# Enigmatisms/NeRF

Hardware: AMD Instinct MI355X
Metric: rays/s (64+128 samples), 800x800 (higher is better)
Workload: dtype bf16

## Files before the change

include/nerf_amd.h:

```cpp
#ifndef NERF_AMD_H
#define NERF_AMD_H

#include <stddef.h>
#include <stdint.h>

#ifdef __cplusplus
extern "C" {
#endif

#define NERF_AMD_OK            0
#define NERF_AMD_EINVAL       -1
#define NERF_AMD_EUNSUPPORTED -2
#define NERF_AMD_EHIP         -3

#define NERF_AMD_F32   0
#define NERF_AMD_BF16  1
#define NERF_AMD_BF16_F8 2

#define NERF_AMD_NET_PROPOSAL 0
#define NERF_AMD_NET_MIP      1
#define NERF_AMD_NET_REF      2
#define NERF_AMD_NET_PROPOSAL_128 3
#define NERF_AMD_PROP_W128 0x100
#define NERF_AMD_NET_MIP_128 4
#define NERF_AMD_FINE_W128 0x200

#define NERF_AMD_ACT_RELU     0
#define NERF_AMD_ACT_IDENTITY 1
#define NERF_AMD_ACT_SOFTPLUS 2

const char* nerf_amd_last_error(void);
int         nerf_amd_version(void);
int         nerf_amd_device_info(int* n_cu, int* arch_is_gfx950);

typedef struct nerf_amd_samples {
    int32_t      mode;
    int32_t      S;
    int64_t      M;
    const float* pts;
    int32_t      pts_stride;
    int32_t      z_stride;
    const float* rays;
    const float* z;
    const float* z_base;
    const float* u;
    float        z_jitter;
    int32_t      H, W;
    float        fx, fy;
    float        pose[12];
    int32_t      contract;
    int32_t      ipe;
    float        ipe_radius;
    const float* ipe_dir_norm;
    uint64_t     rng_seed;
    int64_t      rng_ray_offset;
} nerf_amd_samples;

size_t nerf_amd_packed_bytes(int net, int precision);
int    nerf_amd_pack_weights(int net, int precision, const float* const* weights, const float* const* biases,
                             int n_tensors, void* packed, void* stream);

int nerf_amd_proposal_forward(const void* packed, int precision, const nerf_amd_samples* src,
                              float* density, void* stream);
int nerf_amd_mip_forward(const void* packed, int precision, const nerf_amd_samples* src,
                         float* rgbo, void* stream);

int nerf_amd_mip_forward_composite(const void* packed, int precision, const nerf_amd_samples* src, int white_bkg,
                                   float near, float far, float* rgb, float* depth, float* weights, void* stream);

#define NERF_AMD_REF_SRGB 1
int nerf_amd_ref_forward(const void* packed, int precision, const nerf_amd_samples* src, int ref_flags,
                         float* rgbo, float* normal, void* stream);
int nerf_amd_ref_forward_train(const void* packed, int precision, const nerf_amd_samples* src, int ref_flags, const float* bn_noise,
                               float* rgbo, float* normal, void* stream);


int nerf_amd_positional_encoding(const float* x, int64_t M, int L, float* out, void* stream);

int nerf_amd_ipe_feature(const float* z, const float* rays, int64_t N, int S, int L, float r, const float* dir_norm,
                         float* feat, float* mu, float* mu_t, void* stream);
int nerf_amd_ipe_feature_contracted(const float* z, const float* rays, int64_t N, int S, int L, float r, const float* dir_norm,
                                    float* feat, float* mu, float* mu_t, void* stream);
int nerf_amd_cone_parameters(const float* z, int64_t N, int S, float r, float* mu_t, float* var_t, float* var_r, void* stream);
int nerf_amd_dirs_norm(const float* rays, int64_t N, float* out, void* stream);

int nerf_amd_generate_rays(const float* pose_host, int H, int W, float fx, float fy, int64_t ray_offset, int64_t N,
                           float* rays, void* stream);

int nerf_amd_length2pts(const float* rays, const float* z, int64_t N, int S, float* out, void* stream);

int nerf_amd_sigma_to_weights(const float* sigma, const float* z, const float* dirs, int64_t N, int S, int act,
                              float* w, void* stream);

int nerf_amd_max_blur(const float* w, int64_t N, int S, float alpha, float* out, void* stream);

int nerf_amd_inverse_sample(const float* w, const float* z, const float* u, int64_t N, int C, int K, int sort,
                            float* z_out, int64_t* below, void* stream);

int nerf_amd_sample_pdf(const float* bins, const float* weights, const float* u, int64_t N, int B, int K, float* samples,
                        int64_t* below, int64_t* above, void* stream);

int nerf_amd_pixel_rays(const float* pose_host, float fx, float fy, const int64_t* coords, int64_t N, float* rays, void* stream);

int nerf_amd_sample_training_rays(const float* rgbs, const int64_t* coords, int64_t n_pixels, const float* pose_host, float fx, float fy,
                                  float near, float far, int64_t N, int C, uint64_t rng_seed, float* pts, float* lengths, float* rgb,
                                  float* rays, void* stream);
int nerf_amd_sample_training_rays_dev(const float* rgbs, const int64_t* coords, int64_t n_pixels, const float* pose_dev, float fx, float fy,
                                      float near, float far, int64_t N, int C, const uint64_t* seed_dev, float* pts, float* lengths,
                                      float* rgb, float* rays, void* stream);
int nerf_amd_philox_uniforms(float* out, int64_t N, int K, uint64_t rng_seed, const uint64_t* seed_dev, void* stream);
int nerf_amd_sample_scene_rays(const float* images, const float* poses, int64_t V, int H, int W, const int64_t* view_ids, int64_t K, int x0,
                               int x1, int y0, int y1, float fx, float fy, float near, float far, int64_t N, int C, uint64_t rng_seed,
                               const uint64_t* seed_dev, float* pts, float* lengths, float* rgb, float* rays, int64_t* index, void* stream);
#define NERF_AMD_PHILOX_INV 0
#define NERF_AMD_PHILOX_STRAT 1
int nerf_amd_philox_stream(float* out, int64_t N, int K, uint64_t rng_seed, const uint64_t* seed_dev, int64_t ray_offset, int stream_id,
// ... 151 lines not shown
```

nerf_amd/_lib.py:

```python
import ctypes as C
import os

import torch

_HERE = os.path.dirname(os.path.abspath(__file__))
LIB_PATH = os.environ.get("NERF_AMD_LIB") or os.path.join(_HERE, "libnerf_amd.so")

F32, BF16 = 0, 1
BF16_F8 = 2
EXPECTED_VERSION = 125
NET_PROPOSAL, NET_MIP, NET_REF, NET_PROPOSAL_128, NET_MIP_128 = 0, 1, 2, 3, 4
FINE_W128 = 0x200
PROP_W128 = 0x100
ACT_RELU, ACT_IDENTITY, ACT_SOFTPLUS = 0, 1, 2
SPACING_LINEAR, SPACING_DISPARITY = 0, 1
SPACINGS = {"linear": SPACING_LINEAR, "disparity": SPACING_DISPARITY}

c_float_p = C.POINTER(C.c_float)
c_void = C.c_void_p
i64 = C.c_int64


class Samples(C.Structure):
    _fields_ = [("mode", C.c_int32), ("S", C.c_int32), ("M", C.c_int64), ("pts", c_void), ("pts_stride", C.c_int32),
                ("z_stride", C.c_int32), ("rays", c_void), ("z", c_void), ("z_base", c_void), ("u", c_void),
                ("z_jitter", C.c_float), ("H", C.c_int32), ("W", C.c_int32), ("fx", C.c_float), ("fy", C.c_float),
                ("pose", C.c_float * 12), ("contract", C.c_int32), ("ipe", C.c_int32), ("ipe_radius", C.c_float),
                ("ipe_dir_norm", c_void), ("rng_seed", C.c_uint64), ("rng_ray_offset", C.c_int64)]


SIGNATURES = {
    "nerf_amd_last_error": (C.c_char_p, []),
    "nerf_amd_version": (C.c_int, []),
    "nerf_amd_device_info": (C.c_int, [C.POINTER(C.c_int), C.POINTER(C.c_int)]),
    "nerf_amd_packed_bytes": (C.c_size_t, [C.c_int, C.c_int]),
    "nerf_amd_pack_weights": (C.c_int, [C.c_int, C.c_int, C.POINTER(c_void), C.POINTER(c_void), C.c_int, c_void, c_void]),
    "nerf_amd_proposal_forward": (C.c_int, [c_void, C.c_int, C.POINTER(Samples), c_void, c_void]),
    "nerf_amd_mip_forward": (C.c_int, [c_void, C.c_int, C.POINTER(Samples), c_void, c_void]),
    "nerf_amd_mip_forward_composite": (C.c_int, [c_void, C.c_int, C.POINTER(Samples), C.c_int, C.c_float, C.c_float, c_void, c_void, c_void,
                                                 c_void]),
    "nerf_amd_ref_forward": (C.c_int, [c_void, C.c_int, C.POINTER(Samples), C.c_int, c_void, c_void, c_void]),
    "nerf_amd_ref_forward_train": (C.c_int, [c_void, C.c_int, C.POINTER(Samples), C.c_int, c_void, c_void, c_void, c_void]),
    "nerf_amd_positional_encoding": (C.c_int, [c_void, i64, C.c_int, c_void, c_void]),
    "nerf_amd_ipe_feature": (C.c_int, [c_void, c_void, i64, C.c_int, C.c_int, C.c_float, c_void, c_void, c_void, c_void, c_void]),
    "nerf_amd_ipe_feature_contracted": (C.c_int, [c_void, c_void, i64, C.c_int, C.c_int, C.c_float, c_void, c_void, c_void, c_void, c_void]),
    "nerf_amd_cone_parameters": (C.c_int, [c_void, i64, C.c_int, C.c_float, c_void, c_void, c_void, c_void]),
    "nerf_amd_dirs_norm": (C.c_int, [c_void, i64, c_void, c_void]),
    "nerf_amd_generate_rays": (C.c_int, [c_float_p, C.c_int, C.c_int, C.c_float, C.c_float, i64, i64, c_void, c_void]),
    "nerf_amd_length2pts": (C.c_int, [c_void, c_void, i64, C.c_int, c_void, c_void]),
    "nerf_amd_sigma_to_weights": (C.c_int, [c_void, c_void, c_void, i64, C.c_int, C.c_int, c_void, c_void]),
    "nerf_amd_max_blur": (C.c_int, [c_void, i64, C.c_int, C.c_float, c_void, c_void]),
    "nerf_amd_inverse_sample": (C.c_int, [c_void, c_void, c_void, i64, C.c_int, C.c_int, C.c_int, c_void, c_void, c_void]),
    "nerf_amd_sample_pdf": (C.c_int, [c_void, c_void, c_void, i64, C.c_int, C.c_int, c_void, c_void, c_void, c_void]),
    "nerf_amd_pixel_rays": (C.c_int, [c_float_p, C.c_float, C.c_float, c_void, i64, c_void, c_void]),
    "nerf_amd_sample_training_rays": (C.c_int, [c_void, c_void, i64, c_float_p, C.c_float, C.c_float, C.c_float, C.c_float, i64, C.c_int, C.c_uint64,
                                               c_void, c_void, c_void, c_void, c_void]),
    "nerf_amd_sample_training_rays_dev": (C.c_int, [c_void, c_void, i64, c_void, C.c_float, C.c_float, C.c_float, C.c_float, i64, C.c_int, c_void,
                                                   c_void, c_void, c_void, c_void, c_void]),
    "nerf_amd_sample_scene_rays": (C.c_int, [c_void, c_void, i64, C.c_int, C.c_int, c_void, i64, C.c_int, C.c_int, C.c_int, C.c_int, C.c_float, C.c_float,
                                            C.c_float, C.c_float, i64, C.c_int, C.c_uint64, c_void, c_void, c_void, c_void, c_void, c_void, c_void]),
    "nerf_amd_philox_uniforms": (C.c_int, [c_void, i64, C.c_int, C.c_uint64, c_void, c_void]),
    "nerf_amd_philox_stream": (C.c_int, [c_void, i64, C.c_int, C.c_uint64, c_void, i64, C.c_int, c_void]),
    "nerf_amd_advance_seed": (C.c_int, [c_void, c_void]),
    "nerf_amd_stratified_points": (C.c_int, [c_void, c_void, c_void, C.c_float, i64, C.c_int, c_void, c_void, c_void]),
    "nerf_amd_resample": (C.c_int, [c_void, c_void, c_void, c_void, C.c_float, c_void, C.c_int, c_void, i64, C.c_int,
                                    C.c_int, C.c_int, C.c_float, C.c_uint64, i64, c_void, c_void, c_void, c_void, c_void]),
    "nerf_amd_composite": (C.c_int, [c_void, c_void, C.c_int, c_void, C.c_int, i64, C.c_int, C.c_int, C.c_int, C.c_float, C.c_float,
                                     C.c_float, c_void, c_void, c_void, c_void, c_void, c_void, c_void]),
    "nerf_amd_train_dump_rows_mask_partials": (i64, []),
    "nerf_amd_train_dump_rows_mask": (C.c_int, [c_void, C.c_int, C.c_int, i64, C.c_int, C.c_int, c_void, c_void, c_void, c_void]),
    "nerf_amd_render_ref_workspace_bytes": (C.c_size_t, [i64, C.c_int]),
    "nerf_amd_render_rays_ref": (C.c_int, [c_void, c_void, C.c_int, C.c_int, c_void, C.POINTER(Samples), i64, c_void, c_void, c_void, i64, C.c_int,
                                          C.c_float, C.c_float, C.c_int, c_void, c_void, c_void, c_void, c_void, c_void]),
    "nerf_amd_encode_rows": (C.c_int, [c_void, C.c_int, i64, C.c_int, C.c_int, C.c_int, c_void, c_void]),
    "nerf_amd_merge_depths": (C.c_int, [c_void, c_void, i64, C.c_int, C.c_int, c_void, c_void]),
    "nerf_amd_merge_depths_order": (C.c_int, [c_void, c_void, c_void, i64, C.c_int, C.c_int, c_void, c_void, c_void, c_void]),
    "nerf_amd_coarse_grad_select": (C.c_int, [c_void, c_void, i64, C.c_int, C.c_int, C.c_int, c_void, c_void]),
    "nerf_amd_mfma_stream": (C.c_int, [C.c_int, C.c_int, C.c_int, c_void, c_void]),
    "nerf_amd_weighted_dot_loss": (C.c_int, [c_void, c_void, c_void, i64, C.c_int, C.c_float, c_void, c_void, c_void]),
    "nerf_amd_weighted_dot_loss_backward": (C.c_int, [c_void, c_void, c_void, c_void, i64, C.c_int, C.c_float, c_void, c_void, c_void, c_void]),
    "nerf_amd_distortion_loss": (C.c_int, [c_void, c_void, i64, C.c_int, C.c_int, C.c_float, c_void, c_void, c_void]),
    "nerf_amd_distortion_loss_backward": (C.c_int, [c_void, c_void, i64, C.c_int, C.c_int, C.c_float, c_void, c_void, c_void, c_void]),
    "nerf_amd_get_bounds": (C.c_int, [c_void, c_void, i64, C.c_int, C.c_int, c_void, c_void]),
    "nerf_amd_train_dump_bytes": (C.c_size_t, [C.c_int, C.c_int, i64]),
    "nerf_amd_proposal_forward_train": (C.c_int, [c_void, C.c_int, C.POINTER(Samples), c_void, c_void, c_void]),
    "nerf_amd_mip_forward_train": (C.c_int, [c_void, C.c_int, C.POINTER(Samples), c_void, c_void, c_void]),
    "nerf_amd_train_dump_to_rows": (C.c_int, [c_void, C.c_int, C.c_int, i64, C.c_int, C.c_int, c_void, c_void]),
    "nerf_amd_relu_mask": (C.c_int, [c_void, c_void, C.c_int, i64, c_void]),
    "nerf_amd_relu_mask_bias_partials": (i64, [C.c_int, i64, C.c_int]),
    "nerf_amd_relu_mask_bias": (C.c_int, [c_void, c_void, C.c_int, i64, C.c_int, c_void, c_void]),
    "nerf_amd_packed_backward_bytes": (C.c_size_t, [C.c_int, C.c_int]),
    "nerf_amd_pack_weights_backward": (C.c_int, [C.c_int, C.c_int, C.POINTER(c_void), C.c_int, c_void, c_void]),
    "nerf_amd_proposal_backward_chain": (C.c_int, [c_void, C.c_int, c_void, i64, c_void, c_void, c_void]),
    "nerf_amd_mip_backward_chain": (C.c_int, [c_void, C.c_int, c_void, c_void, i64, c_void, c_void, c_void]),
    "nerf_amd_weight_grads_workspace_bytes": (C.c_size_t, [C.c_int, C.c_int, i64]),
    "nerf_amd_proposal_weight_grads": (C.c_int, [C.c_int, i64, c_void, c_void, C.POINTER(c_void), C.POINTER(c_void), c_void, c_void]),
    "nerf_amd_mip_weight_grads": (C.c_int, [C.c_int, i64, c_void, c_void, C.POINTER(c_void), C.POINTER(c_void), C.POINTER(c_void),
                                           C.POINTER(c_void), c_void, c_void]),
    "nerf_amd_ref_forward_train_dump": (C.c_int, [c_void, C.c_int, C.POINTER(Samples), C.c_int, c_void, c_void, c_void, c_void, c_void, c_void]),
    "nerf_amd_ref_forward_train_dump_rng": (C.c_int, [c_void, C.c_int, C.POINTER(Samples), C.c_int, C.c_uint64, c_void, C.c_float, c_void, c_void, c_void,
                                                      c_void, c_void]),
    "nerf_amd_philox_normal": (C.c_int, [c_void, i64, C.c_uint64, c_void, C.c_float, i64, c_void]),
    "nerf_amd_density_grad_workspace_bytes": (C.c_size_t, [C.c_int, C.c_int, i64]),
    "nerf_amd_density_grad": (C.c_int, [C.c_int, c_void, C.c_int, i64, c_void, c_void, C.c_int, c_void, C.c_int, c_void, c_void, c_void]),
    "nerf_amd_ref_backward_workspace_bytes": (C.c_size_t, [C.c_int, i64]),
    "nerf_amd_ref_backward": (C.c_int, [c_void, C.c_int, C.c_int, i64, c_void, c_void, c_void, C.c_int, c_void, C.c_int, c_void, C.POINTER(c_void),
                                       C.POINTER(c_void), c_void, c_void]),
    "nerf_amd_adam_step": (C.c_int, [C.POINTER(c_void), C.POINTER(c_void), C.POINTER(c_void), C.POINTER(c_void), C.POINTER(i64), C.c_int, c_void,
                                    C.c_double, c_void, C.c_double, C.c_double, C.c_double, C.c_float, c_void]),
    "nerf_amd_sigma_to_weights_backward": (C.c_int, [c_void, c_void, c_void, i64, C.c_int, C.c_int, c_void, c_void, c_void]),
    "nerf_amd_composite_backward": (C.c_int, [c_void, c_void, C.c_int, c_void, C.c_int, i64, C.c_int, C.c_int, C.c_int, C.c_float, C.c_float,
                                              C.c_float, c_void, c_void, c_void, c_void, c_void]),
    "nerf_amd_max_blur_backward": (C.c_int, [c_void, c_void, i64, C.c_int, c_void, c_void]),
    "nerf_amd_get_bounds_backward": (C.c_int, [c_void, c_void, i64, C.c_int, C.c_int, c_void, c_void]),
    "nerf_amd_render_workspace_bytes": (C.c_size_t, [i64, C.c_int]),
    "nerf_amd_render_rays": (C.c_int, [c_void, c_void, C.c_int, c_void, C.POINTER(Samples), i64, c_void, c_void, c_void, i64,
                                       C.c_int, C.c_float, C.c_float, C.c_int, c_void, c_void, c_void, c_void, c_void]),
    "nerf_amd_warp_depths": (C.c_int, [c_void, c_void, i64, C.c_int, C.c_int, C.c_int, C.c_float, C.c_float, c_void, c_void, c_void]),
# ... 49 lines not shown
```

nerf_amd/_packed.py:

```python
from typing import List

import torch

from . import ops


class PackedWeightsMixin:

    _net_id: int = -1

    def _linear_layers(self) -> List[torch.nn.Linear]:
        raise NotImplementedError

    def _layers(self) -> List[torch.nn.Linear]:
        c = self.__dict__.get("_layers_cache")
        if c is None:
            c = self.__dict__["_layers_cache"] = list(self._linear_layers())
        return c

    def _layer_params(self):
        c = self.__dict__.get("_layer_params_cache")
        layers = self._layers()
        if c is None or c[0][0] is not layers[0].weight or c[1][-1] is not layers[-1].bias:
            c = self.__dict__["_layer_params_cache"] = ([l.weight for l in layers], [l.bias for l in layers])
        return c

    def _layers_changed(self) -> None:
        self.__dict__.pop("_layers_cache", None)
        self.__dict__.pop("_layer_params_cache", None)
        self.invalidate_packed()

    def _kernel_weight_shapes(self):
        return None

    def _column_segments(self):
        return None

    @staticmethod
    def encoding_segment(levels: int, cat_origin: bool, kernel_col: int = 0, module_col: int = 0):
        return (kernel_col, module_col, 3 + 6 * levels) if cat_origin else (kernel_col + 3, module_col, 6 * levels)

    def kernel_params(self, shapes=None):
        shapes = self._kernel_weight_shapes() if shapes is None else shapes
        ws, bs = self._layer_params()
        if shapes is None or all(tuple(w.shape) == tuple(s) for w, s in zip(ws, shapes)):
            return list(ws), list(bs)
        pw, pb = [], []
        segs = self._column_segments() or [None] * len(ws)
        with torch.no_grad():
            for w, b, s, seg in zip(ws, bs, shapes, segs):
                if tuple(w.shape) == tuple(s):
                    pw.append(w); pb.append(b)
                    continue
                W = torch.zeros(tuple(s), dtype=w.dtype, device=w.device)
                if seg is None:
                    W[: w.shape[0], : w.shape[1]] = w
                else:
                    for kc, mc, n in seg:
                        W[: w.shape[0], kc: kc + n] = w[:, mc: mc + n]
                B = torch.zeros((s[0],), dtype=b.dtype, device=b.device)
                B[: b.shape[0]] = b
                pw.append(W); pb.append(B)
        return pw, pb

    def unpad_grads(self, gW, gb):
        layers = self._layers()
        segs = self._column_segments() or [None] * len(layers)

        def cols(g, l, seg):
            if tuple(g.shape) == tuple(l.weight.shape):
                return g
            if seg is None:
                return g[: l.weight.shape[0], : l.weight.shape[1]]
            return torch.cat([g[: l.weight.shape[0], kc: kc + n] for kc, _, n in seg], dim=1)
        return ([cols(g, l, seg) for g, l, seg in zip(gW, layers, segs)],
                [g[: l.bias.shape[0]] if tuple(g.shape) != tuple(l.bias.shape) else g for g, l in zip(gb, layers)])

    def _generic(self) -> bool:
        return False

    def grad_sinks(self):
        owner = self.__dict__.get("_grad_owner")
        if owner is None or self._generic():
            return None
        layers = self._layers()
        shapes = self._kernel_weight_shapes()
        if shapes is not None and any(tuple(l.weight.shape) != tuple(sh) for l, sh in zip(layers, shapes)):
            return None
        return owner.sinks_for(self, layers)

    def _narrow_layout(self) -> bool:
        return False

    def _pack_now(self, precision: int, narrow: bool = False) -> torch.Tensor:
        ws, bs = self.kernel_params()
        return ops.pack_weights(self._net_id, precision, ws, bs)

    def packed_backward(self, precision: int) -> torch.Tensor:
        return ops.pack_weights_backward(self._net_id, precision, self.kernel_params()[0])

    def _packed_key(self):
        return (ops.PARAM_GENERATION[0],) + tuple((p.data_ptr(), p._version) for p in self.parameters())

    def invalidate_packed(self) -> None:
        self.__dict__.setdefault("_packed_cache", {}).clear()
        self.__dict__.setdefault("_rows_packed", {}).clear()

    def train(self, mode: bool = True):
        self.invalidate_packed()
        return super().train(mode)

    def packed(self, precision: int, wide: bool = False) -> torch.Tensor:
        narrow = (not wide) and self._narrow_layout()
        cache = self.__dict__.setdefault("_packed_cache", {})
        if self.training:
            cache.clear()
            return self._pack_now(precision, narrow)
        key = self._packed_key()
        hit = cache.get((precision, narrow))
        if hit is None or hit[0] != key:
            blob = self._pack_now(precision, narrow)
            cache[(precision, narrow)] = (key, blob)
            return blob
        return hit[1]


def require_no_grad(*tensors):
    if torch.is_grad_enabled() and any(t is not None and t.requires_grad for t in tensors):
        raise NotImplementedError(
            "nerf_amd: the HIP path is forward-only in this round (backward = SURVEY.md section 8f-1); "
            "wrap the call in torch.no_grad()")
```

nerf_amd/addtional.py:

```python
import torch
from torch import nn
from torch.nn import functional as F

from . import ops
from . import autograd_bridge as ab
from ._packed import PackedWeightsMixin, require_no_grad
from .nerf_helper import makeMLP


def getBounds(weights: torch.Tensor, inds: torch.Tensor):
    if ab.needs_grad(weights):
        return ab.HipOp.apply(lambda w, i: ops.get_bounds(w, i), lambda g, w, i: (ops.get_bounds_backward(i, g, w.shape[-1]), None), 1, weights, inds)
    return ops.get_bounds(weights, inds)


class ProposalLoss(nn.Module):
    def forward(self, prop_bounds: torch.Tensor, nerf_weights: torch.Tensor) -> torch.Tensor:
        return torch.sum(F.relu(nerf_weights - prop_bounds) ** 2 / (nerf_weights + 1e-8))


def _distortion(weights: torch.Tensor, t: torch.Tensor, mode: int, scale: float, expr) -> torch.Tensor:
    if not weights.is_cuda:
        return expr(weights, t) * scale
    if t.shape[-1] > ops.BWD_MAX_SAMPLES:
# ... 16 lines not shown
            dists = dists / dists.norm(dim=-1, keepdim=True)
            avg_weights = (weights[..., :-1] + weights[..., 1:]) / 2.
            delta = fine_ts[..., 1:] - fine_ts[..., :-1]
            return torch.mean(avg_weights[:, None, :] * avg_weights[..., None] * dists) + torch.mean(delta * (avg_weights ** 2)) / 3.
        return _distortion(weights, fine_ts, 0, 1.0, expr)


class DistortionLoss(nn.Module):

    def __init__(self, scale: float = 1.0) -> None:
        super().__init__()
        self.scale = float(scale)

    def forward(self, weights: torch.Tensor, edges: torch.Tensor) -> torch.Tensor:
        def expr(w, e):
            mid = (e[..., :-1] + e[..., 1:]) / 2.
            pair = (w[..., :, None] * w[..., None, :] * torch.abs(mid[..., :, None] - mid[..., None, :])).sum((-2, -1))
            return torch.mean(pair + (w * w * (e[..., 1:] - e[..., :-1])).sum(-1) / 3.)
        return _distortion(weights, edges, 1, self.scale, expr)


class SoftL1Loss(nn.Module):
    def __init__(self, epsilon=0.001) -> None:
        super().__init__()
        self.eps = epsilon

    def forward(self, pred: torch.Tensor, target: torch.Tensor):
        return torch.mean((pred - target) ** 2)


class LossPSNR(nn.Module):
    __LOG_10__ = 2.3025851249694824

    def forward(self, x):
        return -10. * torch.log(x) / LossPSNR.__LOG_10__


class ProposalNetwork(PackedWeightsMixin, nn.Module):
    _net_id = ops.NET_PROPOSAL
    _supports_grad_sinks = True

    @staticmethod
    def init_weight(m):
        if isinstance(m, nn.Linear):
            nn.init.trunc_normal_(m.weight, std=.02)
            if m.bias is not None:
                nn.init.constant_(m.bias, 0)

    def __init__(self, position_flevel, hidden_unit=128, cat_origin=True) -> None:
        super().__init__()
        self.position_dims = position_flevel * 6
        self.position_flevel = position_flevel
        self.cat_origin = cat_origin
        self.hidden_unit = hidden_unit
        in_dim = self.position_dims + (3 if cat_origin else 0)
        self.layers = nn.Sequential(*makeMLP(in_dim, hidden_unit), *makeMLP(hidden_unit, hidden_unit),
                                    *makeMLP(hidden_unit, hidden_unit), *makeMLP(hidden_unit, hidden_unit),
                                    *makeMLP(hidden_unit, 1, None))
        self.apply(self.init_weight)

    def _linear_layers(self):
        return [self.layers[0], self.layers[2], self.layers[4], self.layers[6], self.layers[8]]

    def _check_config(self):
        if not (self.position_flevel >= 1 and self.hidden_unit >= 1):
            raise NotImplementedError("nerf_amd: ProposalNetwork needs position_flevel >= 1 and hidden_unit >= 1")

    def _generic(self) -> bool:
        return self.hidden_unit > 256 or self.position_flevel > 10

    def _column_segments(self):
        if self.position_flevel == 10 and self.cat_origin:
            return None
        return [[self.encoding_segment(self.position_flevel, self.cat_origin)], None, None, None, None]

    def _kernel_weight_shapes(self):
        return [(256, 63), (256, 256), (256, 256), (256, 256), (1, 256)]

    _NARROW_SHAPES = [(128, 63), (128, 128), (128, 128), (128, 128), (1, 128)]

    def _narrow_layout(self) -> bool:
        return self.hidden_unit <= 128

    def _pack_now(self, precision: int, narrow: bool = False) -> torch.Tensor:
        if not narrow:
            return super()._pack_now(precision)
        ws, bs = self.kernel_params(self._NARROW_SHAPES)
        blob = ops.pack_weights(ops.NET_PROPOSAL_128, precision, ws, bs)
        blob._nerf_amd_layout = ops.PROP_W128
        return blob

    def loadFromFile(self, load_path: str, use_amp=False, other_stuff=None):
        save = torch.load(load_path, map_location="cpu")
        own = self.state_dict()
        own.update({k: save["model"][k] for k in own.keys()})
        self.load_state_dict(own)
        if use_amp:
            from apex import amp
            amp.load_state_dict(save["amp"])
        print("NeRF Model loaded from '%s'" % (load_path))
        if other_stuff is not None:
            return [save[k] for k in other_stuff]

    def forward(self, pts: torch.Tensor, encoded_pt: torch.Tensor = None, contract: bool = False) -> torch.Tensor:
        self._check_config()
        if self._generic():
            from . import generic_path
            return generic_path.proposal_forward(self, pts, contract=contract)
        prec = ops.current_precision()
        layers = self._layers()
        params = [l.weight for l in layers] + [l.bias for l in layers]
        if ab.needs_grad(pts, *params):
            if pts.numel() == 0:
                return ops.proposal_forward(self.packed(prec), prec, pts.detach(), contract=contract) + sum(q.sum() for q in params) * 0.0
            from . import mlp_backward
            held = {}
            tprec = prec if pts.requires_grad else ops.train_precision(prec)
            want_pos = bool(pts.requires_grad)

            def hip(p, *wb):
                out, held["dump"] = ops.proposal_forward_train(self.packed(prec, wide=True), tprec, p, contract=contract)
                return out

            def bwd(g, p, *wb):
                if "dump" not in held:
                    raise RuntimeError("nerf_amd: the activation dump of this forward was already consumed (backward twice over the same graph)")
                if "bwd_blob" not in held:
                    held["bwd_blob"] = self.packed_backward(prec)
                if ab._VJP.inputs_only:
                    gx = ops.density_grad(ops.NET_PROPOSAL, held["bwd_blob"], prec, held["dump"], p.reshape(-1, 3), scale=g.reshape(-1), contract=contract)
                    return (gx.view(p.shape), *[None] * len(wb))
                gx = None
                if ab.POSITION_GRADS and want_pos:
                    gx = ops.density_grad(ops.NET_PROPOSAL, held["bwd_blob"], prec, held["dump"], p.reshape(-1, 3), scale=g.reshape(-1), contract=contract).view(p.shape)
                sinks = self.grad_sinks()
                direct = sinks is not None and sinks[2]
                kw = wb[:5]
                gW, gb = mlp_backward.proposal_backward(g.reshape(-1), p.reshape(-1, 3), held.pop("dump"), tprec, kw, packed_bwd=held["bwd_blob"],
                                                        out=(sinks[0], sinks[1]) if direct else None)
                if sinks is not None:
                    if not direct:
                        torch._foreach_add_(list(sinks[0]) + list(sinks[1]), list(gW) + list(gb))
                    return (gx, *[None] * len(wb))
                gW, gb = self.unpad_grads(gW, gb)
                return (gx, *gW, *gb)
            return ab.HipOp.apply(hip, bwd, 1, pts, *params)
        return ops.proposal_forward(self.packed(prec), prec, pts, contract=contract)

    @staticmethod
    def get_weights(density: torch.Tensor, zvals: torch.Tensor, ray_dirs: torch.Tensor = None) -> torch.Tensor:
        if ab.needs_grad(density, zvals):
            if ray_dirs is not None:
                zvals = zvals * ray_dirs.norm(dim=-1, keepdim=True)
            if density.shape[-1] > ops.BWD_MAX_SAMPLES:
                ab.unsupported("a differentiable sigma -> weights row of %d samples (the backward kernel keeps a ray in registers: <= %d)" % (density.shape[-1], ops.BWD_MAX_SAMPLES))
            return ab.HipOp.apply(lambda s, z: ops.sigma_to_weights(s, z, None, ops.ACT_RELU),
                                  lambda g, s, z: (ops.sigma_to_weights_backward(s, z, None, ops.ACT_RELU, g), None), 1, density, zvals)
        return ops.sigma_to_weights(density, zvals, ray_dirs, ops.ACT_RELU)
```

nerf_amd/csrc/capi.hip:

```cpp
#include <hip/hip_runtime.h>
#include <stdio.h>
#include <string.h>

#include "../../include/nerf_amd.h"
#include "mlp_layout.h"

int mlp_launch_proposal(const void*, int, const nerf_amd_samples&, float*, hipStream_t);
int mlp_launch_proposal128(const void*, int, const nerf_amd_samples&, float*, hipStream_t);
int mlp_launch_mip(const void*, int, const nerf_amd_samples&, float*, hipStream_t);
int mlp_launch_mip128(const void*, int, const nerf_amd_samples&, float*, hipStream_t);
int mlp_launch_mip_composite(const void*, int, const nerf_amd_samples&, float*, float*, float*, int, float, float, hipStream_t);
int mlp_launch_ref(const void*, int, const nerf_amd_samples&, float*, float*, const float*, int, hipStream_t);
size_t mlp_train_layer_stride(int, int64_t);
size_t mlp_train_mask_stride(int, int64_t);
int mlp_launch_proposal_train(const void*, int, const nerf_amd_samples&, float*, void*, hipStream_t);
int mlp_launch_mip_train(const void*, int, const nerf_amd_samples&, float*, void*, hipStream_t);
int sk_frag_to_rows(const void*, int, int64_t, int, int64_t, void*, hipStream_t);
int sk_relu_mask(void*, const void*, int, int64_t, hipStream_t);
int sk_merge_sorted(const float*, const float*, int64_t, int, int, float*, hipStream_t);
int sk_merge_sorted_order(const float*, const float*, const int64_t*, int64_t, int, int, float*, int64_t*, int64_t*, hipStream_t);
int sk_coarse_grad_select(const float*, const int64_t*, int64_t, int, int, int, float*, hipStream_t);
int pack_mfma_stream(int, int, int, float*, hipStream_t);
int sk_weighted_dot_loss(const float*, const float*, const float*, int64_t, int, float, float*, float*, hipStream_t);
int sk_weighted_dot_loss_backward(const float*, const float*, const float*, const float*, int64_t, int, float, float*, float*, float*, hipStream_t);
int sk_distortion_loss(const float*, const float*, int64_t, int, int, float, float*, float*, hipStream_t);
int sk_distortion_loss_backward(const float*, const float*, int64_t, int, int, float, const float*, float*, float*, hipStream_t);
int sk_encode_rows(const float*, int, int64_t, int, int, int, void*, hipStream_t);
int sk_frag_rows_mask_blocks();
int sk_frag_rows_mask(const void*, int, int64_t, int, int64_t, void*, void*, float*, hipStream_t);
int sk_relu_mask_bias(void*, const void*, int, int64_t, int, float*, hipStream_t);
int pack_ref(int, const float* const*, const float* const*, void*, hipStream_t);
int pack_proposal_bwd(int, const float* const*, void*, hipStream_t);
int pack_mip_bwd(int, const float* const*, void*, hipStream_t);
int pack_ref_bwd(int, const float* const*, void*, hipStream_t);
int mlp_launch_ref_train(const void*, int, const nerf_amd_samples&, float*, float*, const float*, void*, float*, int, hipStream_t, unsigned long long, const unsigned long long*, float);
size_t bwd_density_grad_workspace_bytes(int, int64_t);
int bwd_density_grad(int, const void*, int, int64_t, const void*, const float*, int, const float*, int, float*, void*, hipStream_t, int);
size_t bwd_ref_workspace_bytes(int, int64_t);
int bwd_ref_backward(const void*, int, int64_t, const void*, const float*, const float*, int, const float*, int, const float*, float* const*,
                     float* const*, void*, int, hipStream_t);
int bwd_launch_prop_chain(const void*, int, const float*, int64_t, const void*, void*, hipStream_t);
int bwd_launch_mip_chain(const void*, int, const float*, const float*, int64_t, const void*, void*, hipStream_t);
size_t bwd_wgrad_workspace_bytes(int, int, int64_t);
int bwd_prop_weight_grads(int, int64_t, const void*, const void*, float* const*, float* const*, void*, hipStream_t);
int bwd_mip_weight_grads(int, int64_t, const void*, const void*, const float* const*, const float* const*, float* const*, float* const*, void*,
                         hipStream_t);
int bwd_launch_adam(float* const*, const float* const*, float* const*, float* const*, const long long*, int, float*, double, const double*, double,
                    double, double, float, hipStream_t);
int pack_proposal(int, const float* const*, const float* const*, void*, hipStream_t);
int pack_proposal128(int, const float* const*, const float* const*, void*, hipStream_t);
int pack_mip128(int, const float* const*, const float* const*, void*, hipStream_t);
int pack_mip(int, const float* const*, const float* const*, void*, hipStream_t);
int sk_positional_encoding(const float*, int64_t, int, float*, hipStream_t);
int sk_ipe_feature(const float*, const float*, int64_t, int, int, float, const float*, float*, float*, float*, int, hipStream_t);
int sk_dirs_norm(const float*, int64_t, float*, hipStream_t);
int sk_dirs_norm_scratch(const float*, int64_t, float*, void*, hipStream_t);
int sk_train_sampler(const float*, const int64_t*, int64_t, const float*, const float*, float, float, float, float, int64_t, int, uint64_t, const uint64_t*,
                     float*, float*, float*, float*, hipStream_t);
int sk_scene_sampler(const float*, const float*, int64_t, int, int, const int64_t*, int64_t, int, int, int, int, float, float, float, float, int64_t, int,
                     uint64_t, const uint64_t*, float*, float*, float*, float*, int64_t*, hipStream_t);
int sk_philox_uniforms(float*, int64_t, int, uint64_t, const uint64_t*, int64_t, int, hipStream_t);
int sk_philox_normal(float*, int64_t, uint64_t, const uint64_t*, float, int64_t, hipStream_t);
size_t gk_gemm_workspace_bytes(int64_t, int64_t, int64_t);
int gk_gemm(int, int64_t, int64_t, int64_t, const float*, int64_t, int64_t, const float*, int64_t, int64_t, float*, int64_t, const float*, int, const float*, int64_t,
            void*, hipStream_t);
int gk_sigmoid_backward(const float*, int64_t, const float*, int64_t, int64_t, int, float*, int64_t, hipStream_t);
int gr_dir_inputs(const float*, int64_t, const float*, int64_t, int64_t, int, const float*, float*, int64_t, float*, hipStream_t);
int gr_dir_inputs_backward(const float*, int64_t, const float*, int64_t, int64_t, int, const float*, const float*, int64_t, const float*, int64_t, float*, int64_t,
                           hipStream_t);
int gr_combine(const float*, int64_t, const float*, int64_t, int64_t, int, float*, hipStream_t);
int gr_combine_backward(const float*, int64_t, const float*, int64_t, const float*, int64_t, int64_t, int, float*, int64_t, float*, int64_t, hipStream_t);
int gr_pe_backward(const float*, int64_t, const float*, int64_t, int64_t, int, int, float*, hipStream_t);
int gr_add_rows(float*, int64_t, const float*, int64_t, int64_t, int, hipStream_t);
int gr_contract(const float*, int64_t, int64_t, const float*, int64_t, float*, hipStream_t);
int rg_rows_gemm(int64_t, int64_t, int64_t, const void*, int64_t, const void*, int64_t, int64_t, const float*, int, void*, int64_t, int, hipStream_t);
int rg_rows_to_bf16(const float*, int64_t, int64_t, int64_t, int, int, void*, int64_t, hipStream_t);
int sk_advance_seed(uint64_t*, hipStream_t);
int sk_cone_parameters(const float*, int64_t, int, float, float*, float*, float*, hipStream_t);
int sk_generate_rays(const float*, int, int, float, float, int64_t, int64_t, float*, hipStream_t);
int sk_length2pts(const float*, const float*, int64_t, int, float*, hipStream_t);
int sk_sigma_to_weights(const float*, const float*, const float*, int64_t, int, int, float*, hipStream_t);
int sk_max_blur(const float*, int64_t, int, float, float*, hipStream_t);
int sk_inverse_sample(const float*, const float*, const float*, int64_t, int, int, int, int, float*, int64_t*, int64_t*, hipStream_t);
int sk_pixel_rays(const float*, float, float, const int64_t*, int64_t, float*, hipStream_t);
int sk_stratified_points(const float*, const float*, const float*, float, int64_t, int, float*, float*, hipStream_t);
int sk_resample(const float*, const float*, const float*, const float*, float, const float*, int, const float*, int64_t, int,
                int, int, float, uint64_t, int64_t, float*, int64_t*, float*, float*, hipStream_t);
int sk_composite(const float*, const float*, int, const float*, int, int64_t, int, int, int, float, float, float, const float*,
                 const float*, float*, float*, float*, float*, hipStream_t);
int sk_get_bounds(const float*, const int64_t*, int64_t, int, int, float*, hipStream_t);
int sk_warp_depths(const float*, const float*, int64_t, int, int, float, float, float, float, float*, float*, hipStream_t);
int sk_warped_stratified(const float*, const float*, int64_t, int, uint64_t, int64_t, float, float, float, float, float*, float*, float*, hipStream_t);
size_t sk_warped_resample_lds_bytes(int, int);
int sk_warped_resample(const float*, const float*, const float*, int, const float*, int64_t, int, int, int, float, float, float, float, float, uint64_t,
                       int64_t, float*, float*, int64_t*, float*, hipStream_t);
int sk_weights_backward(const float*, int, int, const float*, int, const float*, int, int64_t, int, int, int, float, const float*, const float*,
                        const float*, const float*, int, float, float, float*, int, int, float*, hipStream_t);
int sk_max_blur_backward(const float*, const float*, int64_t, int, float*, hipStream_t);
int sk_get_bounds_backward(const int64_t*, const float*, int64_t, int, int, float*, hipStream_t);

namespace {
thread_local char g_err[512] = "";

int fail(int code, const char* fmt, const char* a = "") {
    snprintf(g_err, sizeof(g_err), fmt, a);
    return code;
}
int hip_status(int e, const char* where) {
    if (e == 0) return NERF_AMD_OK;
    snprintf(g_err, sizeof(g_err), "%s: HIP error %d (%s)", where, e, hipGetErrorString((hipError_t)e));
    return NERF_AMD_EHIP;
}
inline hipStream_t S(void* s) { return reinterpret_cast<hipStream_t>(s); }

int check_samples(const nerf_amd_samples* s, bool need_dir) {
    if (!s) return fail(NERF_AMD_EINVAL, "samples descriptor is NULL");
    if (s->M < 0) return fail(NERF_AMD_EINVAL, "negative sample count");
    if (s->mode == 0) {
        if (!s->pts && s->M) return fail(NERF_AMD_EINVAL, "mode 0 needs pts");
        if (s->pts_stride < (need_dir ? 6 : 3)) return fail(NERF_AMD_EINVAL, "pts_stride too small for this network");
    } else if (s->mode == 1 || s->mode == 2) {
        if (s->S <= 0) return fail(NERF_AMD_EINVAL, "S must be positive");
        if (s->mode == 1 && !s->rays && s->M) return fail(NERF_AMD_EINVAL, "mode 1 needs rays");
        if (s->mode == 2 && (s->H <= 0 || s->W <= 0)) return fail(NERF_AMD_EINVAL, "mode 2 needs H, W");
        if (!s->z && !s->z_base && s->M) return fail(NERF_AMD_EINVAL, "need z, or z_base (with u, or without: in-kernel uniforms from rng_seed)");
    } else {
        return fail(NERF_AMD_EINVAL, "unknown sample mode");
    }
    if (s->ipe) {
        if (!need_dir) return fail(NERF_AMD_EUNSUPPORTED, "integrated PE is wired for the MipNeRF kernel only");
        if (s->mode != 1 || !s->z || s->z_stride < s->S + 1) return fail(NERF_AMD_EINVAL, "integrated PE needs mode 1 with S+1 depths per ray (z, z_stride > S)");
        if (!s->ipe_dir_norm || !(s->ipe_radius > 0.0f)) return fail(NERF_AMD_EINVAL, "integrated PE needs ipe_dir_norm (device) and a positive ipe_radius");
    }
    return NERF_AMD_OK;
}
bool bad_prec(int p) { return p != NERF_AMD_F32 && p != NERF_AMD_BF16; }
int check_distortion(int64_t N, int Sn, int mode) {
    if (N < 0) return fail(NERF_AMD_EINVAL, "negative ray count");
    if (mode != 0 && mode != 1) return fail(NERF_AMD_EINVAL, "unknown mode (0: Regularizer, 1: Mip-NeRF 360 L_dist)");
    if (Sn < 2 || Sn > NERF_AMD_DISTORTION_MAX_S) return fail(NERF_AMD_EINVAL, "bad size (S must be 2..1024 depths per row: a ray's rows live in LDS)");
    return NERF_AMD_OK;
}
int check_spacing(int spacing, float near, float far, float* gn, float* gf) {
    if (spacing != NERF_AMD_SPACING_DISPARITY) return fail(NERF_AMD_EINVAL, "unknown spacing (the warped entry points take NERF_AMD_SPACING_DISPARITY only)");
    if (!(near > 0.0f)) return fail(NERF_AMD_EINVAL, "disparity spacing needs near > 0");
    if (!(far > near) || !(far <= 3.0e38f)) return fail(NERF_AMD_EINVAL, "disparity spacing needs near < far (finite)");
    *gn = (float)(1.0 / (double)near);
    *gf = (float)(1.0 / (double)far);
    if (!(*gf < *gn)) return fail(NERF_AMD_EINVAL, "disparity spacing: 1/near and 1/far coincide in fp32");
    return NERF_AMD_OK;
}
int check_warped_resample_shape(int C, int K) {
    if (C < 3 || C > 256 || K < 1 || K > 1024) return fail(NERF_AMD_EINVAL, "need 3 <= C <= 256 and 1 <= K <= 1024");
    if (sk_warped_resample_lds_bytes(C, K) > 65536) return fail(NERF_AMD_EINVAL, "C and K too large: the per-ray rows of four rays must fit 64 KiB of LDS");
    return NERF_AMD_OK;
}
}

extern "C" {

const char* nerf_amd_last_error(void) { return g_err; }
int nerf_amd_version(void) { return 125; }

int nerf_amd_device_info(int* n_cu, int* arch_is_gfx950) {
    int dev = 0;
    hipDeviceProp_t p;
    int e = (int)hipGetDevice(&dev);
    if (!e) e = (int)hipGetDeviceProperties(&p, dev);
    if (e) return hip_status(e, "nerf_amd_device_info");
    if (n_cu) *n_cu = p.multiProcessorCount;
    if (arch_is_gfx950) *arch_is_gfx950 = strncmp(p.gcnArchName, "gfx950", 6) == 0;
    return NERF_AMD_OK;
}

size_t nerf_amd_packed_bytes(int net, int precision) {
    if (bad_prec(precision)) return 0;
    if (net == NERF_AMD_NET_PROPOSAL) return PropLayout::packed_bytes(precision);
    if (net == NERF_AMD_NET_MIP) return MipLayout::packed_bytes(precision);
    if (net == NERF_AMD_NET_REF) return RefLayout::packed_bytes(precision);
    if (net == NERF_AMD_NET_PROPOSAL_128) return PropLayout128::packed_bytes(precision);
    if (net == NERF_AMD_NET_MIP_128) return MipLayout128::packed_bytes(precision);
    return 0;
}
static int launch_mip_any(int flags, const void* packed, int precision, const nerf_amd_samples& s, float* rgbo, hipStream_t st) {
    return (flags & NERF_AMD_FINE_W128) ? mlp_launch_mip128(packed, precision, s, rgbo, st) : mlp_launch_mip(packed, precision, s, rgbo, st);
}
static int launch_proposal_any(int flags, const void* packed, int precision, const nerf_amd_samples& s, float* density, hipStream_t st) {
    return (flags & NERF_AMD_PROP_W128) ? mlp_launch_proposal128(packed, precision, s, density, st) : mlp_launch_proposal(packed, precision, s, density, st);
}

int nerf_amd_pack_weights(int net, int precision, const float* const* weights, const float* const* biases, int n_tensors,
                          void* packed, void* stream) {
    if (bad_prec(precision)) return fail(NERF_AMD_EINVAL, "unknown precision");
    if (!weights || !biases || !packed) return fail(NERF_AMD_EINVAL, "NULL argument");
    const int want = (net == NERF_AMD_NET_PROPOSAL || net == NERF_AMD_NET_PROPOSAL_128) ? 5
                     : ((net == NERF_AMD_NET_MIP || net == NERF_AMD_NET_MIP_128) ? 11 : (net == NERF_AMD_NET_REF ? 20 : -1));
    if (want < 0) return fail(NERF_AMD_EINVAL, "unknown network");
    if (n_tensors != want) return fail(NERF_AMD_EINVAL, "wrong number of weight tensors for this network");
    for (int i = 0; i < want; ++i)
        if (!weights[i] || !biases[i]) return fail(NERF_AMD_EINVAL, "NULL weight or bias tensor");
    const int e = net == NERF_AMD_NET_PROPOSAL ? pack_proposal(precision, weights, biases, packed, S(stream))
                  : net == NERF_AMD_NET_PROPOSAL_128 ? pack_proposal128(precision, weights, biases, packed, S(stream))
                  : net == NERF_AMD_NET_MIP_128 ? pack_mip128(precision, weights, biases, packed, S(stream))
                  : (net == NERF_AMD_NET_MIP ? pack_mip(precision, weights, biases, packed, S(stream))
                                             : pack_ref(precision, weights, biases, packed, S(stream)));
    return hip_status(e, "nerf_amd_pack_weights");
}

int nerf_amd_proposal_forward(const void* packed, int precision, const nerf_amd_samples* src, float* density, void* stream) {
    const int lflags = precision & ~0xff;
    precision &= 0xff;
    if (bad_prec(precision) || (lflags & ~NERF_AMD_PROP_W128)) return fail(NERF_AMD_EINVAL, "unknown precision");
    if (int c = check_samples(src, false)) return c;
    if (src->M == 0) return NERF_AMD_OK;
    if (!packed || !density) return fail(NERF_AMD_EINVAL, "NULL argument");
    return hip_status(launch_proposal_any(lflags, packed, precision, *src, density, S(stream)), "nerf_amd_proposal_forward");
}

int nerf_amd_mip_forward(const void* packed, int precision, const nerf_amd_samples* src, float* rgbo, void* stream) {
    const int lflags = precision & ~0xff;
    precision &= 0xff;
    if (bad_prec(precision) || (lflags & ~NERF_AMD_FINE_W128)) return fail(NERF_AMD_EINVAL, "unknown precision");
    if (int c = check_samples(src, true)) return c;
    if (src->M == 0) return NERF_AMD_OK;
    if (!packed || !rgbo) return fail(NERF_AMD_EINVAL, "NULL argument");
    if ((lflags & NERF_AMD_FINE_W128) && src->ipe) return fail(NERF_AMD_EINVAL, "the 128-wide fine layout has no integrated-PE kernel: pack the network 256-wide");
    return hip_status(launch_mip_any(lflags, packed, precision, *src, rgbo, S(stream)), "nerf_amd_mip_forward");
}

int nerf_amd_mip_forward_composite(const void* packed, int precision, const nerf_amd_samples* src, int white_bkg, float near,
                                   float far, float* rgb, float* depth, float* weights, void* stream) {
    const int lflags = precision & ~0xff;
    precision &= 0xff;
    if (bad_prec(precision) || (lflags & ~NERF_AMD_FINE_W128)) return fail(NERF_AMD_EINVAL, "unknown precision");
    if (lflags & NERF_AMD_FINE_W128)
        return fail(NERF_AMD_EUNSUPPORTED, "the 128-wide fine layout has no fused-compositing kernel: use nerf_amd_mip_forward + nerf_amd_composite");
    if (int c = check_samples(src, true)) return c;
    if (src->mode != 1 || !src->z) return fail(NERF_AMD_EUNSUPPORTED, "fused compositing needs mode 1 (rays + z)");
    if (src->ipe) return fail(NERF_AMD_EUNSUPPORTED, "integrated PE: use nerf_amd_mip_forward + nerf_amd_composite");
    if (src->S != 32 && src->S != 64 && src->S != 128) return fail(NERF_AMD_EUNSUPPORTED, "fused compositing needs S in {32, 64, 128}");
    if (src->M == 0) return NERF_AMD_OK;
    if (!packed || !rgb) return fail(NERF_AMD_EINVAL, "NULL argument");
    return hip_status(mlp_launch_mip_composite(packed, precision, *src, rgb, depth, weights, white_bkg, near, far, S(stream)),
                      "nerf_amd_mip_forward_composite");
}

static bool bad_ref_flags(int f) { return (f & ~NERF_AMD_REF_SRGB) != 0; }
int nerf_amd_ref_forward(const void* packed, int precision, const nerf_amd_samples* src, int ref_flags, float* rgbo, float* normal, void* stream) {
    if (bad_prec(precision) || bad_ref_flags(ref_flags)) return fail(NERF_AMD_EINVAL, "unknown precision or ref_flags");
    if (int c = check_samples(src, true)) return c;
    if (src->M == 0) return NERF_AMD_OK;
    if (!packed || !rgbo) return fail(NERF_AMD_EINVAL, "NULL argument");
    return hip_status(mlp_launch_ref(packed, precision, *src, rgbo, normal, nullptr, ref_flags, S(stream)), "nerf_amd_ref_forward");
}
int nerf_amd_ref_forward_train(const void* packed, int precision, const nerf_amd_samples* src, int ref_flags, const float* bn_noise, float* rgbo,
                               float* normal, void* stream) {
    if (bad_prec(precision) || bad_ref_flags(ref_flags)) return fail(NERF_AMD_EINVAL, "unknown precision or ref_flags");
    if (int c = check_samples(src, true)) return c;
    if (src->M == 0) return NERF_AMD_OK;
    if (!packed || !rgbo || !bn_noise) return fail(NERF_AMD_EINVAL, "NULL argument");
    return hip_status(mlp_launch_ref(packed, precision, *src, rgbo, normal, bn_noise, ref_flags, S(stream)), "nerf_amd_ref_forward_train");
}

int nerf_amd_positional_encoding(const float* x, int64_t M, int L, float* out, void* stream) {
    if (M < 0 || L < 1 || L > 24) return fail(NERF_AMD_EINVAL, "bad M or L");
    if (M && (!x || !out)) return fail(NERF_AMD_EINVAL, "NULL argument");
    return hip_status(sk_positional_encoding(x, M, L, out, S(stream)), "nerf_amd_positional_encoding");
}

int nerf_amd_ipe_feature(const float* z, const float* rays, int64_t N, int Sn, int L, float r, const float* dir_norm, float* feat, float* mu,
                         float* mu_t, void* stream) {
    if (N < 0 || Sn < 0 || L < 1 || L > 15) return fail(NERF_AMD_EINVAL, "bad size or L (1..15)");
    if (N * Sn && (!z || !rays || !dir_norm || !feat)) return fail(NERF_AMD_EINVAL, "NULL argument");
    const float r2 = (float)((double)r * (double)r);
    return hip_status(sk_ipe_feature(z, rays, N, Sn, L, r2, dir_norm, feat, mu, mu_t, 0, S(stream)), "nerf_amd_ipe_feature");
}
int nerf_amd_ipe_feature_contracted(const float* z, const float* rays, int64_t N, int Sn, int L, float r, const float* dir_norm, float* feat, float* mu,
                                    float* mu_t, void* stream) {
    if (N < 0 || Sn < 0 || L < 1 || L > 15) return fail(NERF_AMD_EINVAL, "bad size or L (1..15)");
    if (N * Sn && (!z || !rays || !dir_norm || !feat)) return fail(NERF_AMD_EINVAL, "NULL argument");
    const float r2 = (float)((double)r * (double)r);
    return hip_status(sk_ipe_feature(z, rays, N, Sn, L, r2, dir_norm, feat, mu, mu_t, 1, S(stream)), "nerf_amd_ipe_feature_contracted");
}
int nerf_amd_cone_parameters(const float* z, int64_t N, int Sn, float r, float* mu_t, float* var_t, float* var_r, void* stream) {
    if (N < 0 || Sn < 0) return fail(NERF_AMD_EINVAL, "negative size");
    if (N * Sn && (!z || !mu_t || !var_t || !var_r)) return fail(NERF_AMD_EINVAL, "NULL argument");
    return hip_status(sk_cone_parameters(z, N, Sn, (float)((double)r * (double)r), mu_t, var_t, var_r, S(stream)), "nerf_amd_cone_parameters");
}
int nerf_amd_dirs_norm(const float* rays, int64_t N, float* out, void* stream) {
    if (N < 0 || !out || (N && !rays)) return fail(NERF_AMD_EINVAL, "bad argument");
    return hip_status(sk_dirs_norm(rays, N, out, S(stream)), "nerf_amd_dirs_norm");
}

int nerf_amd_generate_rays(const float* pose_host, int H, int W, float fx, float fy, int64_t ray_offset, int64_t N, float* rays,
                           void* stream) {
// ... 341 lines not shown
    if (bad_prec(precision) || M < 0 || (net != NERF_AMD_NET_PROPOSAL && net != NERF_AMD_NET_REF)) return 0;
    return bwd_density_grad_workspace_bytes(precision, M);
}
int nerf_amd_density_grad(int net, const void* packed_bwd, int precision, int64_t M, const void* act_dump, const float* x, int x_stride,
                          const float* scale, int scale_stride, float* grad, void* workspace, void* stream) {
    const int contract = (net & NERF_AMD_CONTRACTED) ? 1 : 0;
    net &= ~NERF_AMD_CONTRACTED;
    if (bad_prec(precision) || M < 0 || x_stride < 3) return fail(NERF_AMD_EINVAL, "bad precision, size or stride");
    if (net != NERF_AMD_NET_PROPOSAL && net != NERF_AMD_NET_REF) return fail(NERF_AMD_EUNSUPPORTED, "density gradients exist for the proposal and Ref-NeRF networks");
    if (M == 0) return NERF_AMD_OK;
    if (!packed_bwd || !act_dump || !x || !grad || !workspace) return fail(NERF_AMD_EINVAL, "NULL argument");
    return hip_status(bwd_density_grad(net, packed_bwd, precision, M, act_dump, x, x_stride, scale, scale_stride, grad, workspace, S(stream), contract), "nerf_amd_density_grad");
}
size_t nerf_amd_ref_backward_workspace_bytes(int precision, int64_t M) {
    if (bad_prec(precision) || M < 0) return 0;
    return bwd_ref_workspace_bytes(precision, M);
}
int nerf_amd_ref_backward(const void* packed_bwd, int precision, int ref_flags, int64_t M, const void* act_dump, const float* aux, const float* dirs,
                          int dir_stride, const float* g_out, int g_stride, const float* ide_table, float* const* d_weights, float* const* d_biases,
                          void* workspace, void* stream) {
    if (bad_prec(precision) || bad_ref_flags(ref_flags) || M < 0 || dir_stride < 3 || g_stride < 7) return fail(NERF_AMD_EINVAL, "bad precision, flags, size or stride");
    if (!d_weights || !d_biases) return fail(NERF_AMD_EINVAL, "NULL argument");
    for (int i = 0; i < 20; ++i)
        if (!d_weights[i] || !d_biases[i]) return fail(NERF_AMD_EINVAL, "NULL gradient tensor");
    if (M == 0) return fail(NERF_AMD_EINVAL, "no samples (the caller zero-fills the gradients of an empty batch)");
    if (!packed_bwd || !act_dump || !aux || !dirs || !g_out || !ide_table || !workspace) return fail(NERF_AMD_EINVAL, "NULL argument");
    return hip_status(bwd_ref_backward(packed_bwd, precision, M, act_dump, aux, dirs, dir_stride, g_out, g_stride, ide_table, d_weights, d_biases, workspace,
                                       ref_flags, S(stream)), "nerf_amd_ref_backward");
}

int nerf_amd_adam_step(float* const* params, const float* const* grads, float* const* exp_avg, float* const* exp_avg_sq, const int64_t* numel,
                       int n_tensors, float* step, double lr, const double* lr_dev, double beta1, double beta2, double eps, float grad_scale,
                       void* stream) {
    if (n_tensors < 0 || (n_tensors && (!params || !grads || !exp_avg || !exp_avg_sq || !numel)) || !step) return fail(NERF_AMD_EINVAL, "NULL argument");
    for (int i = 0; i < n_tensors; ++i)
        if (numel[i] < 0 || (numel[i] && (!params[i] || !grads[i] || !exp_avg[i] || !exp_avg_sq[i]))) return fail(NERF_AMD_EINVAL, "NULL tensor");
    static_assert(sizeof(long long) == sizeof(int64_t), "int64");
    return hip_status(bwd_launch_adam(params, grads, exp_avg, exp_avg_sq, reinterpret_cast<const long long*>(numel), n_tensors, step, lr, lr_dev,
                                      beta1, beta2, eps, grad_scale, S(stream)), "nerf_amd_adam_step");
}

int nerf_amd_sigma_to_weights_backward(const float* sigma, const float* z, const float* dirs, int64_t N, int Sn, int act,
                                       const float* d_weights, float* d_sigma, void* stream) {
    if (N < 0 || Sn < 1 || Sn > 1024) return fail(NERF_AMD_EINVAL, "bad size (S must be 1..1024)");
    if (N && (!sigma || !z || !d_weights || !d_sigma)) return fail(NERF_AMD_EINVAL, "NULL argument");
    return hip_status(sk_weights_backward(sigma, 1, 0, z, Sn, dirs, 3, N, Sn, dirs ? 1 : 0, act, 0.0f, nullptr, nullptr, d_weights, nullptr, 0, 0.0f,
                                          1.0f, d_sigma, 1, 0, nullptr, S(stream)), "nerf_amd_sigma_to_weights_backward");
}
int nerf_amd_composite_backward(const float* rgbo, const float* z, int z_stride, const float* dirs, int dirs_stride, int64_t N, int Sn,
                                int flags, int act, float sigma_shift, float near, float far, const float* d_rgb,
                                const float* d_weights, const float* d_depth, float* d_rgbo, void* stream) {
    if (N < 0 || Sn < 1 || Sn > 1024 || z_stride < Sn) return fail(NERF_AMD_EINVAL, "bad size (S must be 1..1024)");
    if (N && (!rgbo || !z || !dirs || !d_rgbo)) return fail(NERF_AMD_EINVAL, "NULL argument");
    if (N && !d_rgb) return fail(NERF_AMD_EINVAL, "d_rgb is required (pass zeros when only the weights carry a gradient)");
    return hip_status(sk_weights_backward(rgbo, 4, 3, z, z_stride, dirs, dirs_stride, N, Sn, flags & 1, act, sigma_shift, rgbo, d_rgb, d_weights,
                                          d_depth, (flags >> 1) & 1, near, far, d_rgbo, 4, 3, d_rgbo, S(stream)), "nerf_amd_composite_backward");
}
int nerf_amd_max_blur_backward(const float* weights, const float* d_out, int64_t N, int Sn, float* d_weights, void* stream) {
    if (N < 0 || Sn < 1) return fail(NERF_AMD_EINVAL, "bad size");
    if (N && (!weights || !d_out || !d_weights)) return fail(NERF_AMD_EINVAL, "NULL argument");
    return hip_status(sk_max_blur_backward(weights, d_out, N, Sn, d_weights, S(stream)), "nerf_amd_max_blur_backward");
}
int nerf_amd_get_bounds_backward(const int64_t* below, const float* d_bounds, int64_t N, int C, int K, float* d_w_prop, void* stream) {
    if (N < 0 || C < 1 || C > 4096 || K < 2 || K > 2048) return fail(NERF_AMD_EINVAL, "bad size (C <= 4096, 2 <= K <= 2048)");
    if (N && (!below || !d_bounds || !d_w_prop)) return fail(NERF_AMD_EINVAL, "NULL argument");
    return hip_status(sk_get_bounds_backward(below, d_bounds, N, C, K, d_w_prop, S(stream)), "nerf_amd_get_bounds_backward");
}

size_t nerf_amd_render_workspace_bytes(int64_t N, int n_fine) {
    if (N < 0 || n_fine < 1) return 0;
    const size_t a = ((size_t)N * 64 * 4 + 255) & ~(size_t)255;
    const size_t b = ((size_t)N * (n_fine + 1) * 4 + 255) & ~(size_t)255;
    const size_t c = ((size_t)N * n_fine * 16 + 255) & ~(size_t)255;
    const size_t d = ((size_t)N * 24 + 255) & ~(size_t)255;
    return a + b + c + d + 512;
}

int nerf_amd_render_rays(const void* packed_prop, const void* packed_mip, int precision, const float* rays,
                         const nerf_amd_samples* camera, int64_t ray_offset, const float* z_base, const float* u_strat,
                         const float* u_inv, int64_t N, int n_fine, float near, float far, int white_bkg, float* rgb,
                         float* depth, float* weights, void* workspace, void* stream) {
    const int lflags = precision & ~0xff;
    precision &= 0xff;
    if (bad_prec(precision) || (lflags & ~(NERF_AMD_PROP_W128 | NERF_AMD_FINE_W128))) return fail(NERF_AMD_EINVAL, "unknown precision");
    if ((lflags & NERF_AMD_FINE_W128) && camera && camera->ipe) return fail(NERF_AMD_EINVAL, "the 128-wide fine layout has no integrated-PE kernel: pack the network 256-wide");
    if (N < 0 || n_fine < 1 || n_fine > 1023) return fail(NERF_AMD_EINVAL, "bad N or n_fine");
    if (N == 0) return NERF_AMD_OK;
    if (!packed_prop || !packed_mip || !z_base || !rgb || !workspace) return fail(NERF_AMD_EINVAL, "NULL argument");
    if ((u_strat == nullptr) != (u_inv == nullptr)) return fail(NERF_AMD_EINVAL, "u_strat and u_inv are both given or both NULL (in-kernel uniforms)");
    if (!u_strat && !camera) return fail(NERF_AMD_EINVAL, "in-kernel uniforms need the descriptor (rng_seed, rng_ray_offset)");
    if (!rays && !camera) return fail(NERF_AMD_EINVAL, "need rays or camera");
    const uint64_t seed = camera ? camera->rng_seed : 0;
    const int64_t ray0 = camera ? camera->rng_ray_offset : 0;
    constexpr int C = 64;
    char* ws = reinterpret_cast<char*>((reinterpret_cast<uintptr_t>(workspace) + 255) & ~(uintptr_t)255);
    float* density = reinterpret_cast<float*>(ws);
    ws += ((size_t)N * C * 4 + 255) & ~(size_t)255;
    float* z_fine = reinterpret_cast<float*>(ws);
    ws += ((size_t)N * (n_fine + 1) * 4 + 255) & ~(size_t)255;
    float* rgbo = reinterpret_cast<float*>(ws);
    ws += ((size_t)N * n_fine * 16 + 255) & ~(size_t)255;
    hipStream_t st = S(stream);
    if (!rays) {
        if (camera->H <= 0 || camera->W <= 0 || ray_offset < 0 || ray_offset + N > (int64_t)camera->H * camera->W)
            return fail(NERF_AMD_EINVAL, "ray range outside the camera image");
        float* gen = reinterpret_cast<float*>(ws);
        if (int e = sk_generate_rays(camera->pose, camera->H, camera->W, camera->fx, camera->fy, ray_offset, N, gen, st))
            return hip_status(e, "ray generation");
        rays = gen;
    }
    ws += ((size_t)N * 24 + 255) & ~(size_t)255;
    float* dir_norm = reinterpret_cast<float*>(ws);
    const bool ipe = camera && camera->ipe;
    if (ipe) {
        if (!(camera->ipe_radius > 0.0f)) return fail(NERF_AMD_EINVAL, "integrated PE needs a positive ipe_radius");
        if (camera->ipe_dir_norm) dir_norm = const_cast<float*>(camera->ipe_dir_norm);
        else if (int e = (N >= 8) ? sk_dirs_norm_scratch(rays, N, dir_norm, density, st) : sk_dirs_norm(rays, N, dir_norm, st))
            return hip_status(e, "direction norm");
    }
    const float jitter = (far - near) / (float)n_fine;

    nerf_amd_samples sc{};
    sc.mode = 1; sc.rays = rays; sc.S = C; sc.M = N * C; sc.z = nullptr; sc.z_base = z_base; sc.u = u_strat;
    sc.z_jitter = jitter; sc.z_stride = C;
    sc.contract = camera ? camera->contract : 0;
    sc.rng_seed = seed; sc.rng_ray_offset = ray0;
    if (int e = launch_proposal_any(lflags, packed_prop, precision, sc, density, st)) return hip_status(e, "proposal MLP");
    if (int e = sk_resample(density, nullptr, z_base, u_strat, jitter, rays + 3, 6, u_inv, N, C, n_fine + 1, 0, 0.01f, seed, ray0, z_fine,
                            nullptr, nullptr, nullptr, st)) return hip_status(e, "resample");
    nerf_amd_samples sf{};
    sf.mode = 1; sf.rays = rays; sf.S = n_fine; sf.M = N * n_fine; sf.z = z_fine; sf.z_stride = n_fine + 1;
    sf.contract = sc.contract;
    if (ipe) { sf.ipe = 1; sf.ipe_radius = camera->ipe_radius; sf.ipe_dir_norm = dir_norm; }
    if (int e = launch_mip_any(lflags, packed_mip, precision, sf, rgbo, st)) return hip_status(e, "fine MLP");
    const int flags = 1 | (white_bkg ? 2 : 0);
    if (int e = sk_composite(rgbo, z_fine, n_fine + 1, rays + 3, 6, N, n_fine, flags, NERF_AMD_ACT_RELU, 0.0f, near, far, nullptr,
                             nullptr, rgb, weights, depth, nullptr, st)) return hip_status(e, "composite");
    return NERF_AMD_OK;
}

int nerf_amd_warp_depths(const float* in, const float* rays, int64_t N, int Sn, int inverse, int spacing, float near, float far, float* out, float* pts,
                         void* stream) {
    float gn, gf;
    if (int e = check_spacing(spacing, near, far, &gn, &gf)) return e;
    if (N < 0 || Sn < 1) return fail(NERF_AMD_EINVAL, "need N >= 0 and S >= 1");
    if (N && (!in || !out || (pts && !rays))) return fail(NERF_AMD_EINVAL, "NULL argument");
    if (pts && inverse) return fail(NERF_AMD_EINVAL, "pts are positions o + z d: not with inverse");
    return hip_status(sk_warp_depths(in, rays, N, Sn, inverse ? 1 : 0, near, far, gn, gf, out, pts, S(stream)), "nerf_amd_warp_depths");
}

int nerf_amd_warped_stratified(const float* rays, const float* u, int64_t N, int C, uint64_t rng_seed, int64_t rng_ray_offset, int spacing, float near,
                               float far, float* s_c, float* z_c, float* pts, void* stream) {
    float gn, gf;
    if (int e = check_spacing(spacing, near, far, &gn, &gf)) return e;
    if (N < 0 || C < 3 || C > 256) return fail(NERF_AMD_EINVAL, "need N >= 0 and 3 <= C <= 256");
    if (!u && C > 64) return fail(NERF_AMD_EINVAL, "the stratified Philox stream has 64 slots per ray: pass u for C > 64");
    if (N && (!s_c || !z_c || (pts && !rays))) return fail(NERF_AMD_EINVAL, "NULL argument");
    return hip_status(sk_warped_stratified(rays, u, N, C, rng_seed, rng_ray_offset, near, far, gn, gf, s_c, z_c, pts, S(stream)), "nerf_amd_warped_stratified");
}

int nerf_amd_warped_resample(const float* density, const float* s_c, const float* dirs, int dirs_stride, const float* u_inv, int64_t N, int C, int K,
                             int softplus_density, float blur_alpha, int spacing, float near, float far, uint64_t rng_seed, int64_t rng_ray_offset,
                             float* z_fine, float* s_fine, int64_t* below, float* w_prop, void* stream) {
    float gn, gf;
    if (int e = check_spacing(spacing, near, far, &gn, &gf)) return e;
    if (N < 0) return fail(NERF_AMD_EINVAL, "negative ray count");
    if (int e = check_warped_resample_shape(C, K)) return e;
    if (dirs_stride < 3) return fail(NERF_AMD_EINVAL, "dirs_stride < 3");
    if (N && (!density || !s_c || !dirs || !z_fine)) return fail(NERF_AMD_EINVAL, "NULL argument");
    return hip_status(sk_warped_resample(density, s_c, dirs, dirs_stride, u_inv, N, C, K, softplus_density, blur_alpha, near, far, gn, gf, rng_seed,
                                         rng_ray_offset, z_fine, s_fine, below, w_prop, S(stream)), "nerf_amd_warped_resample");
}

static size_t ws256(size_t bytes) { return (bytes + 255) & ~(size_t)255; }
size_t nerf_amd_render_warped_workspace_bytes(int64_t N, int n_fine) {
    if (N < 0 || n_fine < 1) return 0;
    return 3 * ws256((size_t)N * 64 * 4) + ws256((size_t)N * (n_fine + 1) * 4) + ws256((size_t)N * n_fine * 16) + ws256((size_t)N * 4) + ws256((size_t)N * 24) + 512;
}

int nerf_amd_render_rays_warped(const void* packed_prop, const void* packed_mip, int precision, const float* rays, const nerf_amd_samples* camera,
                                int64_t ray_offset, const float* u_strat, const float* u_inv, int64_t N, int n_fine, int spacing, float near, float far,
                                int white_bkg, float* rgb, float* depth, float* weights, void* workspace, void* stream) {
    const int lflags = precision & ~0xff;
    precision &= 0xff;
    float gn, gf;
    if (int e = check_spacing(spacing, near, far, &gn, &gf)) return e;
    if (bad_prec(precision) || (lflags & ~(NERF_AMD_PROP_W128 | NERF_AMD_FINE_W128))) return fail(NERF_AMD_EINVAL, "unknown precision");
    if ((lflags & NERF_AMD_FINE_W128) && camera && camera->ipe) return fail(NERF_AMD_EINVAL, "the 128-wide fine layout has no integrated-PE kernel: pack the network 256-wide");
    if (N < 0 || n_fine < 1 || n_fine > 1023) return fail(NERF_AMD_EINVAL, "bad N or n_fine");
    constexpr int C = 64;
    if (int e = check_warped_resample_shape(C, n_fine + 1)) return e;
    if (N == 0) return NERF_AMD_OK;
    if (!packed_prop || !packed_mip || !rgb || !workspace) return fail(NERF_AMD_EINVAL, "NULL argument");
    if ((u_strat == nullptr) != (u_inv == nullptr)) return fail(NERF_AMD_EINVAL, "u_strat and u_inv are both given or both NULL (in-kernel uniforms)");
    if (!u_strat && !camera) return fail(NERF_AMD_EINVAL, "in-kernel uniforms need the descriptor (rng_seed, rng_ray_offset)");
    if (!rays && !camera) return fail(NERF_AMD_EINVAL, "need rays or camera");
    const bool ipe = camera && camera->ipe;
    if (ipe && !(camera->ipe_radius > 0.0f)) return fail(NERF_AMD_EINVAL, "integrated PE needs a positive ipe_radius");
    if (ipe && !rays) return fail(NERF_AMD_EINVAL, "integrated PE needs an explicit ray table");
    if (!rays && (camera->H <= 0 || camera->W <= 0 || ray_offset < 0 || ray_offset + N > (int64_t)camera->H * camera->W))
        return fail(NERF_AMD_EINVAL, "ray range outside the camera image");
    const uint64_t seed = camera ? camera->rng_seed : 0;
    const int64_t ray0 = camera ? camera->rng_ray_offset : 0;
    char* ws = reinterpret_cast<char*>((reinterpret_cast<uintptr_t>(workspace) + 255) & ~(uintptr_t)255);
    auto take = [&](size_t bytes) { float* p = reinterpret_cast<float*>(ws); ws += ws256(bytes); return p; };
    float* density = take((size_t)N * C * 4);
    float* s_c = take((size_t)N * C * 4);
    float* z_c = take((size_t)N * C * 4);
    float* z_fine = take((size_t)N * (n_fine + 1) * 4);
    float* rgbo = take((size_t)N * n_fine * 16);
    float* depth_raw = take((size_t)N * 4);
    float* gen = take((size_t)N * 24);
    float* dir_norm = reinterpret_cast<float*>(ws);
    hipStream_t st = S(stream);
    if (!rays) {
        if (int e = sk_generate_rays(camera->pose, camera->H, camera->W, camera->fx, camera->fy, ray_offset, N, gen, st))
            return hip_status(e, "ray generation");
        rays = gen;
    }
    if (ipe) {
        if (camera->ipe_dir_norm) dir_norm = const_cast<float*>(camera->ipe_dir_norm);
        else if (int e = (N >= 8) ? sk_dirs_norm_scratch(rays, N, dir_norm, density, st) : sk_dirs_norm(rays, N, dir_norm, st))
            return hip_status(e, "direction norm");
    }
    if (int e = sk_warped_stratified(rays, u_strat, N, C, seed, ray0, near, far, gn, gf, s_c, z_c, nullptr, st)) return hip_status(e, "warped stratified draw");
    nerf_amd_samples sc{};
    sc.mode = 1; sc.rays = rays; sc.S = C; sc.M = N * C; sc.z = z_c; sc.z_stride = C;
    sc.contract = camera ? camera->contract : 0;
    if (int e = launch_proposal_any(lflags, packed_prop, precision, sc, density, st)) return hip_status(e, "proposal MLP");
    if (int e = sk_warped_resample(density, s_c, rays + 3, 6, u_inv, N, C, n_fine + 1, 0, 0.01f, near, far, gn, gf, seed, ray0, z_fine, nullptr, nullptr,
                                   nullptr, st)) return hip_status(e, "warped resample");
    nerf_amd_samples sf{};
    sf.mode = 1; sf.rays = rays; sf.S = n_fine; sf.M = N * n_fine; sf.z = z_fine; sf.z_stride = n_fine + 1;
    sf.contract = sc.contract;
    if (ipe) { sf.ipe = 1; sf.ipe_radius = camera->ipe_radius; sf.ipe_dir_norm = dir_norm; }
    if (int e = launch_mip_any(lflags, packed_mip, precision, sf, rgbo, st)) return hip_status(e, "fine MLP");
    const int flags = 1 | (white_bkg ? 2 : 0);
    if (int e = sk_composite(rgbo, z_fine, n_fine + 1, rays + 3, 6, N, n_fine, flags, NERF_AMD_ACT_RELU, 0.0f, 0.0f, 1.0f, nullptr, nullptr, rgb, weights,
                             depth ? depth_raw : nullptr, nullptr, st)) return hip_status(e, "composite");
    if (depth) {
        if (int e = sk_warp_depths(depth_raw, nullptr, N, 1, 1, near, far, gn, gf, depth, nullptr, st)) return hip_status(e, "depth un-warp");
    }
    return NERF_AMD_OK;
}

static size_t ref_ws_part(size_t bytes) { return (bytes + 255) & ~(size_t)255; }
size_t nerf_amd_render_ref_workspace_bytes(int64_t N, int n_fine) {
    if (N < 0 || n_fine < 1) return 0;
    const size_t n = (size_t)N, S = (size_t)n_fine + 64;
    return ref_ws_part(n * 64 * 4) * 2 + ref_ws_part(n * (n_fine + 1) * 4) + ref_ws_part(n * S * 4) + ref_ws_part(n * S * 16) + ref_ws_part(n * S * 12) +
           n * 24 + 256;
}

int nerf_amd_render_rays_ref(const void* packed_prop, const void* packed_ref, int precision, int ref_flags, const float* rays,
                             const nerf_amd_samples* camera, int64_t ray_offset, const float* z_base, const float* u_strat,
                             const float* u_inv, int64_t N, int n_fine, float near, float far, int white_bkg, const float* cam_dir,
                             float* rgb, float* depth, float* normal_img, void* workspace, void* stream) {
    const int lflags = precision & ~0xff;
    precision &= 0xff;
    if (bad_prec(precision) || (lflags & ~NERF_AMD_PROP_W128) || bad_ref_flags(ref_flags)) return fail(NERF_AMD_EINVAL, "unknown precision or ref_flags");
    if (N < 0 || n_fine < 1 || n_fine > 1023) return fail(NERF_AMD_EINVAL, "bad N or n_fine");
    if (N == 0) return NERF_AMD_OK;
    if (!packed_prop || !packed_ref || !z_base || !rgb || !workspace) return fail(NERF_AMD_EINVAL, "NULL argument");
    if ((u_strat == nullptr) != (u_inv == nullptr)) return fail(NERF_AMD_EINVAL, "u_strat and u_inv are both given or both NULL (in-kernel uniforms)");
    if (!u_strat && !camera) return fail(NERF_AMD_EINVAL, "in-kernel uniforms need the descriptor (rng_seed, rng_ray_offset)");
    if (!rays && !camera) return fail(NERF_AMD_EINVAL, "need rays or camera");
    const uint64_t seed = camera ? camera->rng_seed : 0;
    const int64_t ray0 = camera ? camera->rng_ray_offset : 0;
    if ((normal_img != nullptr) != (cam_dir != nullptr)) return fail(NERF_AMD_EINVAL, "normal_img and cam_dir go together");
    const int contract = camera ? camera->contract : 0;
    constexpr int C = 64;
    const int S_all = n_fine + C;
    char* ws = reinterpret_cast<char*>((reinterpret_cast<uintptr_t>(workspace) + 255) & ~(uintptr_t)255);
    auto take = [&](size_t bytes) { float* p = reinterpret_cast<float*>(ws); ws += ref_ws_part(bytes); return p; };
    float* density = take((size_t)N * C * 4);
    float* z_fine = take((size_t)N * (n_fine + 1) * 4);
    float* z_coarse = take((size_t)N * C * 4);
    float* z_all = take((size_t)N * S_all * 4);
    float* rgbo = take((size_t)N * S_all * 16);
    float* normals = take((size_t)N * S_all * 12);
    hipStream_t st = S(stream);
    if (!rays) {
        if (camera->H <= 0 || camera->W <= 0 || ray_offset < 0 || ray_offset + N > (int64_t)camera->H * camera->W)
            return fail(NERF_AMD_EINVAL, "ray range outside the camera image");
        float* gen = reinterpret_cast<float*>(ws);
        if (int e = sk_generate_rays(camera->pose, camera->H, camera->W, camera->fx, camera->fy, ray_offset, N, gen, st))
            return hip_status(e, "ray generation");
        rays = gen;
    }
    const float jitter = (far - near) / (float)n_fine;
    nerf_amd_samples sc{};
    sc.mode = 1; sc.rays = rays; sc.S = C; sc.M = N * C; sc.z = nullptr; sc.z_base = z_base; sc.u = u_strat;
    sc.z_jitter = jitter; sc.z_stride = C;
    sc.contract = contract;
    sc.rng_seed = seed; sc.rng_ray_offset = ray0;
    if (int e = launch_proposal_any(lflags, packed_prop, precision, sc, density, st)) return hip_status(e, "proposal MLP");
    if (int e = sk_resample(density, nullptr, z_base, u_strat, jitter, rays + 3, 6, u_inv, N, C, n_fine + 1, 0, 0.01f, seed, ray0, z_fine,
                            nullptr, nullptr, z_coarse, st)) return hip_status(e, "resample");
    if (int e = sk_merge_sorted(z_fine, z_coarse, N, n_fine + 1, C, z_all, st)) return hip_status(e, "depth merge");
    nerf_amd_samples sf{};
    sf.mode = 1; sf.rays = rays; sf.S = S_all; sf.M = N * S_all; sf.z = z_all; sf.z_stride = S_all;
    sf.contract = contract;
    if (int e = mlp_launch_ref(packed_ref, precision, sf, rgbo, normal_img ? normals : nullptr, nullptr, ref_flags, st)) return hip_status(e, "Ref-NeRF MLP");
    const int flags = 1 | (white_bkg ? 2 : 0);
    if (int e = sk_composite(rgbo, z_all, S_all, rays + 3, 6, N, S_all, flags, NERF_AMD_ACT_SOFTPLUS, 0.5f, near, far,
                             normal_img ? normals : nullptr, cam_dir, rgb, nullptr, depth, normal_img, st)) return hip_status(e, "composite");
    return NERF_AMD_OK;
}

size_t nerf_amd_gemm_workspace_bytes(int64_t M, int64_t N, int64_t P) {
    if (M <= 0 || N <= 0 || P <= 0) return 0;
    return gk_gemm_workspace_bytes(M, N, P);
}

int nerf_amd_gemm(int precision, int64_t M, int64_t N, int64_t P, const float* A, int64_t a_si, int64_t a_sp, const float* B, int64_t b_sp, int64_t b_sj,
                  float* C, int64_t ldc, const float* bias, int act, const float* mask, int64_t ldm, void* workspace, void* stream) {
    if (precision != NERF_AMD_F32 && precision != NERF_AMD_BF16) return fail(NERF_AMD_EINVAL, "nerf_amd_gemm: precision must be NERF_AMD_F32 or NERF_AMD_BF16");
    if (M < 0 || N < 0 || P < 0 || N > 65535LL * 128) return fail(NERF_AMD_EINVAL, "nerf_amd_gemm: bad size");
    if (M == 0 || N == 0) return 0;
    if (!C || (P && (!A || !B))) return fail(NERF_AMD_EINVAL, "nerf_amd_gemm: NULL argument");
    if ((a_si != 1 && a_sp != 1) || (b_sp != 1 && b_sj != 1)) return fail(NERF_AMD_EINVAL, "nerf_amd_gemm: one stride of each operand must be 1");
    if (ldc < N || (mask && ldm < N)) return fail(NERF_AMD_EINVAL, "nerf_amd_gemm: row stride smaller than N");
    if (act < 0 || act > 2) return fail(NERF_AMD_EINVAL, "nerf_amd_gemm: act must be 0 (none), 1 (ReLU) or 2 (sigmoid)");
    if (gk_gemm_workspace_bytes(M, N, P) && !workspace) return fail(NERF_AMD_EINVAL, "nerf_amd_gemm: this shape needs nerf_amd_gemm_workspace_bytes of workspace");
    return hip_status(gk_gemm(precision == NERF_AMD_BF16, M, N, P, A, a_si, a_sp, B, b_sp, b_sj, C, ldc, bias, act, mask, ldm, workspace, S(stream)), "nerf_amd_gemm");
}

int nerf_amd_sigmoid_backward(const float* g, int64_t g_stride, const float* y, int64_t y_stride, int64_t M, int cols, float* out, int64_t out_stride,
                              void* stream) {
    if (M < 0 || cols < 0) return fail(NERF_AMD_EINVAL, "nerf_amd_sigmoid_backward: bad size");
    if (M * cols && (!g || !y || !out)) return fail(NERF_AMD_EINVAL, "nerf_amd_sigmoid_backward: NULL argument");
    if (g_stride < cols || y_stride < cols || out_stride < cols) return fail(NERF_AMD_EINVAL, "nerf_amd_sigmoid_backward: row stride smaller than cols");
    return hip_status(gk_sigmoid_backward(g, g_stride, y, y_stride, M, cols, out, out_stride, S(stream)), "nerf_amd_sigmoid_backward");
}

int nerf_amd_ref_dir_inputs(const float* heads, int64_t heads_stride, const float* dirs, int64_t dirs_stride, int64_t M, int ide_level, const float* ide_table,
                            float* out, int64_t out_stride, float* normal, void* stream) {
    if (M < 0 || ide_level < 1 || ide_level > 5) return fail(NERF_AMD_EINVAL, "nerf_amd_ref_dir_inputs: bad size / ide_level (1..5)");
    if (M && (!heads || !dirs || !ide_table || !out || !normal)) return fail(NERF_AMD_EINVAL, "nerf_amd_ref_dir_inputs: NULL argument");
    const int T = (1 << ide_level) - 1 + ide_level;
    if (heads_stride < 11 || dirs_stride < 3 || out_stride < 2 * T + 1) return fail(NERF_AMD_EINVAL, "nerf_amd_ref_dir_inputs: row stride too small");
    return hip_status(gr_dir_inputs(heads, heads_stride, dirs, dirs_stride, M, ide_level, ide_table, out, out_stride, normal, S(stream)), "nerf_amd_ref_dir_inputs");
}
// ... 77 lines not shown
```

nerf_amd/csrc/mlp_core.h:

```cpp
#pragma once
#include "device_common.h"
#include "host_common.h"
#include "mlp_layout.h"

extern __shared__ __attribute__((aligned(16))) char smem[];

namespace {


struct PBF16 {
    using BReg = bf16x8;
    static constexpr int PREC = NERF_AMD_BF16;
    static constexpr int NW = MLP_NW_BF16;
    static constexpr int NT = 1;
    static constexpr int FRAG_BYTES = 1024;
    static constexpr int FPC = MLP_CHUNK_BYTES / FRAG_BYTES;
    using AReg = bf16x8;
    static constexpr int DEPTH = 4;
    static DEVINL AReg load_a(uint32_t frag_addr) { return *reinterpret_cast<const bf16x8*>(smem + frag_addr); }
    static DEVINL f32x16 mma(const AReg& a, const BReg& b, f32x16 acc) {
        return __builtin_amdgcn_mfma_f32_32x32x16_bf16(a, b, acc, 0, 0, 0);
    }
    template <int POS>
    static DEVINL f32x16 mma_pos(const AReg& a, const BReg& b, f32x16 acc) {
        return __builtin_amdgcn_mfma_f32_32x32x16_bf16(a, b, acc, 0, 0, 0);
    }
    static DEVINL void set(BReg& r, int e, float v) { r[e] = (__bf16)v; }
    template <bool RELU>
    static DEVINL BReg from_acc(const f32x16& acc, int off) {
        typedef __attribute__((ext_vector_type(2))) __bf16 bf16x2;
        BReg r;
#pragma unroll
        for (int e = 0; e < 4; ++e) {
            const f32x2 v = {acc[off + 2 * e], acc[off + 2 * e + 1]};
            const bf16x2 p = __builtin_convertvector(v, bf16x2);
            r[2 * e] = p[0]; r[2 * e + 1] = p[1];
        }
        if (RELU) {
            typedef __attribute__((ext_vector_type(8))) short s16x8;
            s16x8 v = __builtin_bit_cast(s16x8, r);
            const s16x8 zero = {0, 0, 0, 0, 0, 0, 0, 0};
            v = __builtin_elementwise_max(v, zero);
            r = __builtin_bit_cast(BReg, v);
        }
        return r;
    }
    static constexpr bool FAST_PE = true;
    static constexpr int BREG_LDS = 1024;
    static DEVINL void stash(uint32_t addr, const BReg& r) { *reinterpret_cast<bf16x8*>(smem + addr) = r; }
    static DEVINL BReg unstash(uint32_t addr) { return *reinterpret_cast<const bf16x8*>(smem + addr); }
    static DEVINL void store_global(char* block, int lane, const BReg& r) {
        __builtin_nontemporal_store(__builtin_bit_cast(f32x4, r), reinterpret_cast<f32x4*>(block + lane * 16));
    }
    static DEVINL BReg load_global(const char* block, int lane) { return *reinterpret_cast<const bf16x8*>(block + lane * 16); }
};

struct PBF16W : PBF16 {
    static constexpr int NW = 4;
    static constexpr int NT = 2;
};

struct PBF16N : PBF16 {
    static constexpr int NW = 4;
    static constexpr int NT = 3;
};

struct PF32 {
    using BReg = f32x8;
    static constexpr int PREC = NERF_AMD_F32;
    static constexpr int NW = MLP_NW_F32;
    static constexpr int NT = 1;
    static constexpr int FRAG_BYTES = 2048;
    static constexpr int FPC = MLP_CHUNK_BYTES / FRAG_BYTES;
    struct AReg { f32x4 lo, hi; };
    static constexpr int DEPTH = 2;
    static DEVINL AReg load_a(uint32_t frag_addr) {
        AReg a;
        a.lo = *reinterpret_cast<const f32x4*>(smem + frag_addr);
        a.hi = *reinterpret_cast<const f32x4*>(smem + frag_addr + 1024);
        return a;
    }
    static DEVINL f32x16 mma(const AReg& a, const BReg& b, f32x16 acc) {
#pragma unroll
        for (int e = 0; e < 4; ++e) acc = __builtin_amdgcn_mfma_f32_32x32x2f32(a.lo[e], b[e], acc, 0, 0, 0);
#pragma unroll
        for (int e = 0; e < 4; ++e) acc = __builtin_amdgcn_mfma_f32_32x32x2f32(a.hi[e], b[4 + e], acc, 0, 0, 0);
        return acc;
    }
    template <int POS>
    static DEVINL f32x16 mma_pos(const AReg& a, const BReg& b, f32x16 acc) { return mma(a, b, acc); }
    static DEVINL void set(BReg& r, int e, float v) { r[e] = v; }
    template <bool RELU>
    static DEVINL BReg from_acc(const f32x16& acc, int off) {
        BReg r;
#pragma unroll
        for (int e = 0; e < 8; ++e) r[e] = RELU ? fmaxf(acc[off + e], 0.0f) : acc[off + e];
        return r;
    }
    static constexpr bool FAST_PE = false;
    static constexpr int BREG_LDS = 2048;
    static DEVINL void stash(uint32_t addr, const BReg& r) {
        f32x4 lo = {r[0], r[1], r[2], r[3]}, hi = {r[4], r[5], r[6], r[7]};
        *reinterpret_cast<f32x4*>(smem + addr) = lo;
        *reinterpret_cast<f32x4*>(smem + addr + 1024) = hi;
    }
    static DEVINL BReg unstash(uint32_t addr) {
        const f32x4 lo = *reinterpret_cast<const f32x4*>(smem + addr), hi = *reinterpret_cast<const f32x4*>(smem + addr + 1024);
        BReg r = {lo[0], lo[1], lo[2], lo[3], hi[0], hi[1], hi[2], hi[3]};
        return r;
    }
    static DEVINL void store_global(char* block, int lane, const BReg& r) {
        f32x4 lo = {r[0], r[1], r[2], r[3]}, hi = {r[4], r[5], r[6], r[7]};
        __builtin_nontemporal_store(lo, reinterpret_cast<f32x4*>(block + lane * 16));
        __builtin_nontemporal_store(hi, reinterpret_cast<f32x4*>(block + 1024 + lane * 16));
    }
    static DEVINL BReg load_global(const char* block, int lane) {
        const f32x4 lo = *reinterpret_cast<const f32x4*>(block + lane * 16), hi = *reinterpret_cast<const f32x4*>(block + 1024 + lane * 16);
        BReg r = {lo[0], lo[1], lo[2], lo[3], hi[0], hi[1], hi[2], hi[3]};
        return r;
    }
};

typedef __attribute__((ext_vector_type(4))) uint32_t u32x4;
typedef __attribute__((ext_vector_type(2))) uint32_t u32x2;
typedef __attribute__((ext_vector_type(2))) short s16x2;
typedef __attribute__((ext_vector_type(2))) __bf16 bf16x2;
typedef __attribute__((ext_vector_type(2))) unsigned short u16x2;

template <bool SIGNED>
DEVINL uint32_t f8_group_exponent(const bf16x8& v) {
    const u32x4 d = __builtin_bit_cast(u32x4, v);
    uint32_t a = d[0], b = d[1], c = d[2], e = d[3];
    if (SIGNED) { a &= 0x7fff7fffu; b &= 0x7fff7fffu; c &= 0x7fff7fffu; e &= 0x7fff7fffu; }
    const u16x2 m01 = __builtin_elementwise_max(__builtin_bit_cast(u16x2, a), __builtin_bit_cast(u16x2, b));
    const u16x2 m23 = __builtin_elementwise_max(__builtin_bit_cast(u16x2, c), __builtin_bit_cast(u16x2, e));
    const uint32_t m = __builtin_bit_cast(uint32_t, __builtin_elementwise_max(m01, m23));
    const uint32_t top = (m & 0xffffu) > (m >> 16) ? (m & 0xffffu) : (m >> 16);
    const uint32_t ex = top >> 7;
    return ex > 8u ? ex - 7u : 1u;
}
DEVINL u32x2 f8_encode_group(const bf16x8& v, uint32_t E) {
    const float scale = __builtin_bit_cast(float, E << 23);
    const u32x4 d = __builtin_bit_cast(u32x4, v);
    s16x2 lo = {0, 0}, hi = {0, 0};
    lo = __builtin_amdgcn_cvt_scalef32_pk_fp8_bf16(lo, __builtin_bit_cast(bf16x2, (uint32_t)d[0]), scale, false);
    lo = __builtin_amdgcn_cvt_scalef32_pk_fp8_bf16(lo, __builtin_bit_cast(bf16x2, (uint32_t)d[1]), scale, true);
    hi = __builtin_amdgcn_cvt_scalef32_pk_fp8_bf16(hi, __builtin_bit_cast(bf16x2, (uint32_t)d[2]), scale, false);
    hi = __builtin_amdgcn_cvt_scalef32_pk_fp8_bf16(hi, __builtin_bit_cast(bf16x2, (uint32_t)d[3]), scale, true);
    u32x2 r = {__builtin_bit_cast(uint32_t, lo), __builtin_bit_cast(uint32_t, hi)};
    return r;
}
DEVINL bf16x8 f8_decode_group(uint32_t lo, uint32_t hi, uint32_t E) {
    const float scale = __builtin_bit_cast(float, E << 23);
    const bf16x2 p0 = __builtin_amdgcn_cvt_scalef32_pk_bf16_fp8(lo, scale, false), p1 = __builtin_amdgcn_cvt_scalef32_pk_bf16_fp8(lo, scale, true);
    const bf16x2 p2 = __builtin_amdgcn_cvt_scalef32_pk_bf16_fp8(hi, scale, false), p3 = __builtin_amdgcn_cvt_scalef32_pk_bf16_fp8(hi, scale, true);
    bf16x8 r = {p0[0], p0[1], p1[0], p1[1], p2[0], p2[1], p3[0], p3[1]};
    return r;
}
DEVINL void f8_store_group(char* sub_base, int kg, int lane, const u32x2& v, uint32_t E, uint32_t scale_rec) {
    u32x2* dst = reinterpret_cast<u32x2*>(sub_base + (kg >> 1) * 1024 + lane * 16 + (kg & 1) * 8);
    __builtin_nontemporal_store(v, dst);
    *reinterpret_cast<unsigned char*>(smem + scale_rec + lane * 16 + kg) = (unsigned char)E;
}
DEVINL void f8_flush_scales(char* sub_base, int lane, uint32_t scale_rec) {
    const f32x4 v = *reinterpret_cast<const f32x4*>(smem + scale_rec + lane * 16);
    *reinterpret_cast<f32x4*>(sub_base + F8_SCALE_OFF + lane * 16) = v;
}

struct NoResident {
    static constexpr int N = 0;
    static constexpr bool resident(int) { return false; }
    static constexpr int slot(int) { return 0; }
    static constexpr int stream(int f) { return f; }
};
template <int NFRAGS, int PRE, int SUF, int HOLE_A = 0, int HOLE_N = 0>
struct ResidentSet {
    static constexpr int N = PRE + HOLE_N + SUF, N_STREAM = NFRAGS - N;
    static constexpr int FIRST = PRE;
    static constexpr int HOLE_AT = HOLE_A - PRE;
    static constexpr int HOLE_FRAGS = HOLE_N;
    static constexpr int wrap(int f) { return f >= NFRAGS ? f - NFRAGS : f; }
    static constexpr bool in_hole(int f) { return f >= HOLE_A && f < HOLE_A + HOLE_N; }
// ... 181 lines not shown
        prev.template emit<KG * PER + I>();
        emit_step<NKG, KG, Prev, I + 1>(prev);
    }
}

DEVINL f32x16 load_bias(uint32_t addr) {
    f32x16 v;
#pragma unroll
    for (int q = 0; q < 4; ++q) {
        const f32x4 b4 = *reinterpret_cast<const f32x4*>(smem + addr + 32 * q);
        v[4 * q] = b4[0]; v[4 * q + 1] = b4[1]; v[4 * q + 2] = b4[2]; v[4 * q + 3] = b4[3];
    }
    return v;
}
template <class P, int NKG, int FRAG0, int KG, bool MORE, class WS, class InF, class Prev>
DEVINL void pair_k(WS& ws, f32x16 (&acc0)[P::NT], f32x16 (&acc1)[P::NT], f32x16 (&nb)[2], uint32_t next_bias, InF& in, const Prev& prev) {
    if constexpr (KG < NKG) {
        typename P::BReg b[P::NT];
#pragma unroll
        for (int t = 0; t < P::NT; ++t) b[t] = in(KG, t);
        const typename P::AReg a0 = ws.template next<FRAG0 + 2 * KG>();
        constexpr int POS = (KG == 0) ? 0 : ((KG == NKG - 1) ? 2 : 1);
#pragma unroll
        for (int t = 0; t < P::NT; ++t) acc0[t] = P::template mma_pos<POS>(a0, b[t], acc0[t]);
        const typename P::AReg a1 = ws.template next<FRAG0 + 2 * KG + 1>();
#pragma unroll
        for (int t = 0; t < P::NT; ++t) acc1[t] = P::template mma_pos<POS>(a1, b[t], acc1[t]);
        emit_step<NKG, KG>(prev);
        if constexpr (MORE && KG == (NKG > 3 ? NKG - 3 : 0)) {
            nb[0] = load_bias(next_bias);
            nb[1] = load_bias(next_bias + 128);
        }
        pair_k<P, NKG, FRAG0, KG + 1, MORE>(ws, acc0, acc1, nb, next_bias, in, prev);
    }
}
template <class P, int NKG, int FRAG0, int KG, class WS, class InF, class Prev>
DEVINL void single_k(WS& ws, f32x16 (&acc0)[P::NT], f32x16 (&acc1)[P::NT], InF& in, const Prev& prev) {
    if constexpr (KG < NKG) {
        const typename P::AReg a = ws.template next<FRAG0 + KG>();
        constexpr int LAST_EVEN = ((NKG - 1) / 2) * 2, LAST_ODD = (NKG % 2 == 0) ? NKG - 1 : NKG - 2;
#pragma unroll
        for (int t = 0; t < P::NT; ++t) {
            if constexpr (KG % 2 == 0) acc0[t] = P::template mma_pos<(KG == 0) ? 0 : ((KG == LAST_EVEN) ? 2 : 1)>(a, in(KG, t), acc0[t]);
            else acc1[t] = P::template mma_pos<(KG == 1) ? 4 : ((KG == LAST_ODD) ? 2 : 1)>(a, in(KG, t), acc1[t]);
        }
        emit_step<NKG, KG>(prev);
        single_k<P, NKG, FRAG0, KG + 1>(ws, acc0, acc1, in, prev);
    }
}
template <class T, class = void> struct has_group_hook { static constexpr bool value = false; };
template <class T> struct has_group_hook<T, decltype(void(static_cast<T*>(nullptr)->begin_group(0)))> { static constexpr bool value = true; };

template <class P, int NKG, int NFB, int START, int G, bool ZB, class WS, class InF, class OutF, class Prev>
DEVINL auto dense_group(WS& ws, uint32_t bias_lane, f32x16 (&cb)[2], InF& in, OutF& out, const Prev& prev) {
    static_assert(2 * G < NFB, "group index");
    constexpr int FRAG0 = START + 2 * G * NKG;
    constexpr f32x16 zero = {0.0f, 0.0f, 0.0f, 0.0f, 0.0f, 0.0f, 0.0f, 0.0f, 0.0f, 0.0f, 0.0f, 0.0f, 0.0f, 0.0f, 0.0f, 0.0f};
    if constexpr (has_group_hook<OutF>::value) out.begin_group(G);
    if constexpr (2 * G + 1 < NFB) {
        Deferred<P, 2 * G, 2> d;
#pragma unroll
        for (int t = 0; t < P::NT; ++t) {
            if constexpr (ZB) { d.acc[0][t] = zero; d.acc[1][t] = zero; }
            else { d.acc[0][t] = cb[0]; d.acc[1][t] = cb[1]; }
        }
        f32x16 nb[2];
        constexpr bool MORE = 2 * (G + 1) < NFB;
        pair_k<P, NKG, FRAG0, 0, MORE && !ZB>(ws, d.acc[0], d.acc[1], nb, bias_lane + 256 * (G + 1), in, prev);
        if constexpr (MORE) return dense_group<P, NKG, NFB, START, G + 1, ZB>(ws, bias_lane, nb, in, out, prev_of(d, out));
        else return d;
    } else {
        Deferred<P, 2 * G, 1> d;
        f32x16 acc1[P::NT];
#pragma unroll
        for (int t = 0; t < P::NT; ++t) { if constexpr (ZB) d.acc[0][t] = zero; else d.acc[0][t] = cb[0]; acc1[t] = zero; }
        single_k<P, NKG, FRAG0, 0>(ws, d.acc[0], acc1, in, prev);
#pragma unroll
        for (int t = 0; t < P::NT; ++t)
#pragma unroll
            for (int r = 0; r < 16; ++r) d.acc[0][t][r] += acc1[t][r];
        return d;
    }
}
template <class P, int NKG, int NFB, int START, bool ZB = false, class WS, class InF, class OutF, class Prev>
DEVINL auto dense(WS& ws, uint32_t bias_lds, InF&& in, OutF&& out, const Prev& prev) {
    static_assert(START % P::DEPTH == 0 && (NKG * NFB) % P::DEPTH == 0, "layers must start on a prefetch-queue boundary");
    const uint32_t bias_lane = bias_lds + 16 * (lane_id() >> 5);
    f32x16 cb[2];
    if constexpr (!ZB) {
        cb[0] = load_bias(bias_lane);
        if constexpr (NFB > 1) cb[1] = load_bias(bias_lane + 128);
    }
    return dense_group<P, NKG, NFB, START, 0, ZB>(ws, bias_lane, cb, in, out, prev);
}

}
```

nerf_amd/csrc/mlp_kernels.hip:

```cpp
#include "mlp_core.h"

namespace {

template <class P, int L, int NKG>
DEVINL void encode(float x, float y, float z, int h, typename P::BReg (&B)[NKG]) {
    if constexpr (P::FAST_PE) {
        float sv[3], cv[3];
        sincos_quadrant(x, sv[0], cv[0]); sincos_quadrant(y, sv[1], cv[1]); sincos_quadrant(z, sv[2], cv[2]);
#pragma unroll
        for (int f = 0; f < L; ++f) {
#pragma unroll
            for (int c = 0; c < 3; ++c) {
                const int q = 3 * f + c;
                P::set(B[q >> 3], q & 7, h ? cv[c] : sv[c]);
                if (f + 1 < L) {
                    const float s2 = 2.0f * sv[c];
                    const float ns = s2 * cv[c];
                    const float nc = __builtin_fmaf(-s2, sv[c], 1.0f);
                    sv[c] = ns; cv[c] = nc;
                }
            }
        }
#pragma unroll
        for (int q = 3 * L; q < 8 * NKG; ++q) {
// ... 223 lines not shown
    const float* b = reinterpret_cast<const float*>(reinterpret_cast<const char*>(packed) + stream_bytes);
    float* dst = reinterpret_cast<float*>(smem + lds_off);
    for (int i = threadIdx.x; i < n_bias; i += blockDim.x) dst[i] = b[i];
    __syncthreads();
}

struct ActDump {
    char* base;
    unsigned long long layer_stride;
    char* mask_base;
    unsigned long long mask_layer_stride;
};
template <class P>
DEVINL void dump_breg(const ActDump& d, int layer, int64_t subtile, int kg, int lane, const typename P::BReg& r) {
#ifndef ABL_NODUMPST
    P::store_global(d.base + (size_t)layer * d.layer_stride + ((size_t)subtile * 16 + kg) * (size_t)P::BREG_LDS, lane, r);
#endif
}

template <class P> constexpr uint32_t lds_maskacc() { return lds_total<P>(); }
template <class P> constexpr uint32_t lds_total_train() { return lds_total<P>() + P::NW * 2 * P::NT * 1024; }
template <class P> constexpr uint32_t lds_scaleacc() { return lds_total_train<P>(); }
template <class P> constexpr uint32_t lds_total_train_f8() { return lds_total_train<P>() + P::NW * 2 * P::NT * 1024; }
template <class P, bool F8>
DEVINL void dump_hidden(const ActDump& d, uint32_t sacc_wave, int layer, int64_t subtile, int t, int kg, int lane, const typename P::BReg& r) {
    if constexpr (F8) {
        const uint32_t E = f8_group_exponent<false>(r);
        f8_store_group(d.base + (size_t)layer * d.layer_stride + (size_t)subtile * F8_SUB_BYTES, kg, lane, f8_encode_group(r, E), E,
                       sacc_wave + ((layer & 1) * P::NT + t) * 1024);
    } else {
        dump_breg<P>(d, layer, subtile, kg, lane, r);
    }
}
DEVINL uint32_t breg_bits(const bf16x8& v) {
    typedef __attribute__((ext_vector_type(4))) uint32_t u32x4;
    const u32x4 d = __builtin_bit_cast(u32x4, v);
    uint32_t m = 0;
#pragma unroll
    for (int i = 0; i < 4; ++i) {
        const uint32_t x = d[i];
        uint32_t on;
        asm("v_pk_min_u16 %0, %1, %2" : "=v"(on) : "v"(x), "v"(0x00010001u));
        m |= on << i;
    }
    return m;
}
DEVINL uint32_t breg_bits(const f32x8& v) {
    uint32_t m = 0;
#pragma unroll
    for (int e = 0; e < 8; ++e) m |= (v[e] > 0.0f ? 1u : 0u) << ((e >> 1) + 16 * (e & 1));
    return m;
}
template <class P>
DEVINL void mask_or(uint32_t acc_wave, int layer, int t, int kg, int lane, const typename P::BReg& v) {
    unsigned* w = reinterpret_cast<unsigned*>(smem + acc_wave + ((layer & 1) * P::NT + t) * 1024 + lane * 16 + (kg >> 2) * 4);
    __hip_atomic_fetch_or(w, breg_bits(v) << (4 * (kg & 3)), __ATOMIC_RELAXED, __HIP_MEMORY_SCOPE_WORKGROUP);
}
template <class P, bool F8 = false>
DEVINL void mask_flush(const ActDump& d, uint32_t acc_wave, int layer, int64_t sub0, int lane, uint32_t sacc_wave = 0) {
    asm volatile("" ::: "memory");
#pragma unroll
    for (int t = 0; t < P::NT; ++t) {
        f32x4* rec = reinterpret_cast<f32x4*>(smem + acc_wave + ((layer & 1) * P::NT + t) * 1024 + lane * 16);
        const f32x4 v = *rec;
        *reinterpret_cast<f32x4*>(d.mask_base + (size_t)layer * d.mask_layer_stride + (size_t)(sub0 + t) * 1024 + lane * 16) = v;
        *rec = f32x4{0.0f, 0.0f, 0.0f, 0.0f};
        if constexpr (F8)
            f8_flush_scales(d.base + (size_t)layer * d.layer_stride + (size_t)(sub0 + t) * F8_SUB_BYTES, lane, sacc_wave + ((layer & 1) * P::NT + t) * 1024);
    }
    asm volatile("" ::: "memory");
}
template <class P>
DEVINL void mask_acc_init(uint32_t acc_wave, int lane) {
#pragma unroll
    for (int i = 0; i < 2 * P::NT; ++i) *reinterpret_cast<f32x4*>(smem + acc_wave + i * 1024 + lane * 16) = f32x4{0.0f, 0.0f, 0.0f, 0.0f};
}

template <class P, bool TRAIN, bool F8 = false>
__global__ __launch_bounds__(P::NW * 64) void proposal_kernel(const void* __restrict__ packed, nerf_amd_samples s,
                                                              float* __restrict__ density, ActDump dump) {
    using L = PropLayout;
    using BReg = typename P::BReg;
    constexpr int FPC = P::FPC;
    constexpr bool RES = MLP_RESIDENT_PROP && same_type<P, PBF16W>::value && !TRAIN;
    using R = typename conditional_type<RES, PropResident::R, NoResident>::type;
    using WS = typename conditional_type<RES, WeightStream<P, PropResident::NSLOT, R, PropResident::RES>, WeightStream<P, MLP_NSLOT>>::type;
    constexpr uint32_t bias0 = RES ? PropResident::BIAS : MLP_RING_BYTES;
    load_biases(packed, L::stream_bytes(P::PREC), L::N_BIAS, bias0);
    WS ws;
    ws.init(packed, (L::N_FRAGS - R::N) / FPC);
    const int lane = lane_id(), h = lane >> 5, j = lane & 31;
    const int wave = __builtin_amdgcn_readfirstlane((int)(threadIdx.x >> 6));
    constexpr int NT = P::NT;
    constexpr int TS = P::NW * NT * 32;
    const int64_t n_tiles = (s.M + TS - 1) / TS;
    const uint32_t macc = lds_maskacc<P>() + wave * 2 * NT * 1024;
    const uint32_t sacc = lds_scaleacc<P>() + wave * 2 * NT * 1024;
    if constexpr (TRAIN) mask_acc_init<P>(macc, lane);

    for (int64_t tile = blockIdx.x; tile < n_tiles; tile += gridDim.x) {
        int64_t m[NT];
        BReg enc[NT][4];
        if constexpr (NT == 2 && P::FAST_PE) {
            m[0] = tile * TS + (wave * NT) * 32 + j;
            m[1] = m[0] + 32;
            const int64_t mo = h ? m[1] : m[0];
            const Sample sm = fetch_sample(s, mo < s.M ? mo : s.M - 1, false);
            encode_pair<P, 10, 4>(sm.x, sm.y, sm.z, enc[0], enc[1]);
            half_swap_groups<4>(enc[0], enc[1]);
            if constexpr (TRAIN) {
#pragma unroll
                for (int t = 0; t < NT; ++t)
#pragma unroll
                    for (int k = 0; k < 4; ++k) dump_breg<P>(dump, 4, tile * (TS / 32) + wave * NT + t, k, lane, enc[t][k]);
            }
        } else {
#pragma unroll
        for (int t = 0; t < NT; ++t) {
            m[t] = tile * TS + (wave * NT + t) * 32 + j;
            const Sample sm = fetch_sample(s, m[t] < s.M ? m[t] : s.M - 1, false);
            encode<P, 10, 4>(sm.x, sm.y, sm.z, h, enc[t]);
            if constexpr (TRAIN) {
#pragma unroll
                for (int k = 0; k < 4; ++k) dump_breg<P>(dump, 4, tile * (TS / 32) + wave * NT + t, k, lane, enc[t][k]);
            }
        }
        }
        BReg a[NT][16], b[NT][16];
        int lay = 0, lay_pend = 0;
        const int64_t sub0 = tile * (TS / 32) + wave * NT;
        auto put = [&](BReg (&buf)[NT][16], int layer, int fb, int t, const f32x16& acc, int half) {
            buf[t][2 * fb + half] = to_breg_half<P, true>(acc, half);
            if constexpr (TRAIN) {
                dump_hidden<P, F8>(dump, sacc, layer, sub0 + t, t, 2 * fb + half, lane, buf[t][2 * fb + half]);
                mask_or<P>(macc, layer, t, 2 * fb + half, lane, buf[t][2 * fb + half]);
            }
        };
        auto OA = [&](int fb, int t, const f32x16& acc, int half) { put(a, lay, fb, t, acc, half); };
        auto OB = [&](int fb, int t, const f32x16& acc, int half) { put(b, lay, fb, t, acc, half); };
        auto OA_pend = [&](int fb, int t, const f32x16& acc, int half) { put(a, lay_pend, fb, t, acc, half); };
        auto OB_pend = [&](int fb, int t, const f32x16& acc, int half) { put(b, lay_pend, fb, t, acc, half); };
        auto IN_A = [&](int kg, int t) -> BReg { return a[t][kg]; };
        Deferred<P, 6, 2> d = dense<P, 4, 8, L::START[0]>(ws, bias0 + L::BIAS_OFF[0] * 4,
            [&](int kg, int t) -> BReg { return enc[t][kg]; }, OA, NoPrev{});
        static_assert(same_stream_shape<R, FPC>(L::START[1], L::START[3], 128 + P::DEPTH), "chunk parity (in stream space) of the shared a -> b instance");
        auto IN_B = [&](int kg, int t) -> BReg { return b[t][kg]; };
#pragma unroll 1
        for (int r = 0; r < 2; ++r) {
            lay_pend = lay; lay = 1 + 2 * r;
            d = dense<P, 16, 8, L::START[1]>(ws, bias0 + (L::BIAS_OFF[1] + r * 512) * 4, IN_A, OB, prev_of(d, OA_pend));
            if constexpr (TRAIN) mask_flush<P, F8>(dump, macc, lay_pend, sub0, lane, sacc);
            if (r == 0) {
                lay_pend = lay; lay = 2;
                d = dense<P, 16, 8, L::START[2]>(ws, bias0 + L::BIAS_OFF[2] * 4, IN_B, OA, prev_of(d, OB_pend));
                if constexpr (TRAIN) mask_flush<P, F8>(dump, macc, lay_pend, sub0, lane, sacc);
            }
        }
        lay_pend = lay;
        float dens[NT];
        auto OH = [&](int, int t, const f32x16& acc, int half) { if (half == 0) dens[t] = acc[0]; };
        dense<P, 16, 1, L::START[4]>(ws, bias0 + L::BIAS_OFF[4] * 4, IN_B, OH, prev_of(d, OB_pend)).flush(OH);
        if constexpr (TRAIN) mask_flush<P, F8>(dump, macc, lay_pend, sub0, lane, sacc);
#pragma unroll
        for (int t = 0; t < NT; ++t)
            if (h == 0 && m[t] < s.M) density[m[t]] = dens[t];
    }
    ws.drain();
}

constexpr uint32_t lds_total_narrow() { return MLP_RING_BYTES + 9216; }
template <class P>
__global__ __launch_bounds__(P::NW * 64) void proposal128_kernel(const void* __restrict__ packed, nerf_amd_samples s, float* __restrict__ density) {
    using L = PropLayout128;
    using BReg = typename P::BReg;
    constexpr int HK = L::HK, HFB = L::HFB;
    load_biases(packed, L::stream_bytes(P::PREC), L::N_BIAS);
    WeightStream<P, MLP_NSLOT> ws;
    ws.init(packed, L::N_FRAGS / P::FPC);
    const int lane = lane_id(), h = lane >> 5, j = lane & 31;
    const int wave = __builtin_amdgcn_readfirstlane((int)(threadIdx.x >> 6));
    constexpr int NT = P::NT;
    constexpr int TS = P::NW * NT * 32;
    const int64_t n_tiles = (s.M + TS - 1) / TS;
    const uint32_t bias0 = MLP_RING_BYTES;
    for (int64_t tile = blockIdx.x; tile < n_tiles; tile += gridDim.x) {
        int64_t m[NT];
        BReg a[NT][HK], b[NT][HK];
        auto OA = [&](int fb, int t, const f32x16& acc, int half) { a[t][2 * fb + half] = to_breg_half<P, true>(acc, half); };
        auto OB = [&](int fb, int t, const f32x16& acc, int half) { b[t][2 * fb + half] = to_breg_half<P, true>(acc, half); };
        auto IN_A = [&](int kg, int t) -> BReg { return a[t][kg]; };
        auto IN_B = [&](int kg, int t) -> BReg { return b[t][kg]; };
        Deferred<P, HFB - 2, 2> d;
        {
            BReg enc[NT][4];
            constexpr int PAIRED = (NT >= 2 && P::FAST_PE) ? 2 : 0;
#pragma unroll
            for (int t = 0; t < NT; ++t) m[t] = tile * TS + (wave * NT + t) * 32 + j;
            if constexpr (PAIRED) {
                const int64_t mo = h ? m[1] : m[0];
                const Sample sm = fetch_sample(s, mo < s.M ? mo : s.M - 1, false);
                encode_pair<P, 10, 4>(sm.x, sm.y, sm.z, enc[0], enc[1]);
                half_swap_groups<4>(enc[0], enc[1]);
            }
#pragma unroll
            for (int t = PAIRED; t < NT; ++t) {
                const Sample sm = fetch_sample(s, m[t] < s.M ? m[t] : s.M - 1, false);
                encode<P, 10, 4>(sm.x, sm.y, sm.z, h, enc[t]);
            }
            d = dense<P, 4, HFB, L::START[0]>(ws, bias0 + L::BIAS_OFF[0] * 4, [&](int kg, int t) -> BReg { return enc[t][kg]; }, OA, NoPrev{});
        }
        d = dense<P, HK, HFB, L::START[1]>(ws, bias0 + L::BIAS_OFF[1] * 4, IN_A, OB, prev_of(d, OA));
        d = dense<P, HK, HFB, L::START[2]>(ws, bias0 + L::BIAS_OFF[2] * 4, IN_B, OA, prev_of(d, OB));
        d = dense<P, HK, HFB, L::START[3]>(ws, bias0 + L::BIAS_OFF[3] * 4, IN_A, OB, prev_of(d, OA));
        float dens[NT];
        auto OH = [&](int, int t, const f32x16& acc, int half) { if (half == 0) dens[t] = acc[0]; };
        dense<P, HK, 1, L::START[4]>(ws, bias0 + L::BIAS_OFF[4] * 4, IN_B, OH, prev_of(d, OB)).flush(OH);
        skip_frags<P, L::USED_FRAGS, L::N_FRAGS - L::USED_FRAGS>(ws);
#pragma unroll
        for (int t = 0; t < NT; ++t)
            if (h == 0 && m[t] < s.M) density[m[t]] = dens[t];
    }
    ws.drain();
}

struct FusedComposite {
    float* rgb;
    float* depth;
    float* weights;
    int white_bkg;
    float near, far;
};

template <class P, bool TRAIN, bool IPE = false, bool F8 = false, bool FUSED = false>
__global__ __launch_bounds__(P::NW * 64) void mip_kernel(const void* __restrict__ packed, nerf_amd_samples s,
                                                         float* __restrict__ rgbo, FusedComposite fc, ActDump dump) {
    using L = MipLayout;
    using BReg = typename P::BReg;
    constexpr int FPC = P::FPC;
#ifdef MLP_CLOCKPROBE
    const uint64_t probe_c0 = __builtin_readcyclecounter(), probe_r0 = __builtin_amdgcn_s_memrealtime();
#endif
    if constexpr (FUSED) { if (threadIdx.x < 16) reinterpret_cast<unsigned*>(smem + lds_tile<P>() + P::NW * P::NT * 32 * 32 + P::NW * P::NT * 8)[threadIdx.x] = 0u; }
    constexpr bool RES = MLP_RESIDENT_MIP && same_type<P, PBF16W>::value && !TRAIN && !IPE && !F8 && !FUSED;
    using R = typename conditional_type<RES, MipResident::R, NoResident>::type;
    using WS = typename conditional_type<RES, WeightStream<P, MipResident::NSLOT, R, MipResident::RES>, WeightStream<P, MLP_NSLOT>>::type;
    constexpr uint32_t bias0 = RES ? MipResident::BIAS : LDS_BIAS;
    constexpr uint32_t stash_lds = RES ? MipResident::STASH : LDS_STASH, dirs_lds = RES ? MipResident::DIR : lds_dir<P>();
    load_biases(packed, L::stream_bytes(P::PREC), L::N_BIAS, bias0);
// ... 571 lines not shown
#pragma unroll 1
        for (int r = 0; r < 2; ++r) {
            lay_pend = lay; lay = 10 + 2 * r;
            d = dense<P, 16, 8, L::START[10]>(ws, bias0 + (L::BIAS_OFF[10] + 2 * r * 256) * 4, IN_A, OB, prev_of(d, OA_pend));
            if (r == 0) {
                lay_pend = lay; lay = 11;
                d = dense<P, 16, 8, L::START[11]>(ws, bias0 + L::BIAS_OFF[11] * 4, IN_B, OA, prev_of(d, OB_pend));
            }
        }
        lay_pend = lay; lay = 13;
        d = dense<P, 27, 8, L::START[13]>(ws, bias0 + L::BIAS_OFF[13] * 4,
            [&](int kg, int t) -> BReg { if (kg < 11) return P::unstash(stash(t) + kg * P::BREG_LDS); return b[t][kg >= 11 ? kg - 11 : 0]; },
            OA, prev_of(d, OB_pend));
#pragma unroll 1
        for (int r = 0; r < 2; ++r) {
            lay_pend = lay; lay = 14 + 2 * r;
            d = dense<P, 16, 8, L::START[14]>(ws, bias0 + (L::BIAS_OFF[14] + 2 * r * 256) * 4, IN_A, OB, prev_of(d, OA_pend));
            if (r == 0) {
                lay_pend = lay; lay = 15;
                d = dense<P, 16, 8, L::START[15]>(ws, bias0 + L::BIAS_OFF[15] * 4, IN_B, OA, prev_of(d, OB_pend));
            }
        }
        lay_pend = lay;
        float sr[NT], sg[NT], sb[NT];
        auto OSPEC = [&](int, int t, const f32x16& acc, int half) { if (half == 0) { sr[t] = acc[0]; sg[t] = acc[1]; sb[t] = acc[2]; } };
        dense<P, 16, 1, L::START[17]>(ws, bias0 + L::BIAS_OFF[17] * 4, IN_B, OSPEC, prev_of(d, OB_pend)).flush(OSPEC);
#pragma unroll
        for (int t = 0; t < NT; ++t) {
            const float d0 = __shfl(keep[t][0], j + 32, 64), d1 = __shfl(keep[t][1], j + 32, 64), d2 = __shfl(keep[t][2], j + 32, 64),
                        dens = __shfl(keep[t][3], j + 32, 64);
            if (h == 0 && m[t] < s.M) {
                auto sig = [](float v) { return 1.0f / (1.0f + expf(-v)); };
                f32x4 o;
                if (flags & NERF_AMD_REF_SRGB) {
                    o[0] = srgb_from_linear(sig(sr[t]) * sig(keep[t][0]) + sig(d0 - SRGB_LOG3));
                    o[1] = srgb_from_linear(sig(sg[t]) * sig(keep[t][1]) + sig(d1 - SRGB_LOG3));
                    o[2] = srgb_from_linear(sig(sb[t]) * sig(keep[t][2]) + sig(d2 - SRGB_LOG3));
                } else {
                    o[0] = sig(sr[t]) * sig(keep[t][0]) + sig(d0);
                    o[1] = sig(sg[t]) * sig(keep[t][1]) + sig(d1);
                    o[2] = sig(sb[t]) * sig(keep[t][2]) + sig(d2);
                }
                o[3] = dens;
                *reinterpret_cast<f32x4*>(rgbo + m[t] * 4) = o;
                if constexpr (TRAIN) { float* ax = aux + m[t] * 16; ax[11] = sr[t]; ax[12] = sg[t]; ax[13] = sb[t]; ax[14] = 0.0f; ax[15] = 0.0f; }
            }
        }
    }
    ws.drain();
}

int grid_for(int64_t n_tiles) {
    const int n_cu = nerf_host::cu_count();
    return (int)(n_tiles < n_cu ? n_tiles : n_cu);
}

int allow_dynamic_lds(const void* fn, size_t lds) { return nerf_host::allow_dynamic_lds(fn, lds); }

template <class P, class Lay, bool TRAIN = false, bool F8 = false, size_t LDS_FIXED = 0, class K, class... Extra>
int launch(K kernel, const void* packed, const nerf_amd_samples& s, float* out, hipStream_t st, Extra... extra) {
    constexpr int TS = P::NW * P::NT * 32;
    const int64_t n_tiles = (s.M + TS - 1) / TS;
    if (n_tiles == 0) return 0;
    const size_t lds = LDS_FIXED ? LDS_FIXED : (F8 ? lds_total_train_f8<P>() : (TRAIN ? lds_total_train<P>() : lds_total<P>()));
    if (int e = allow_dynamic_lds(reinterpret_cast<const void*>(kernel), lds)) return e;
    hipLaunchKernelGGL(kernel, dim3(grid_for(n_tiles)), dim3(P::NW * 64), lds, st, packed, s, out, extra...);
    return (int)hipGetLastError();
}
const ActDump NO_DUMP{nullptr, 0ull, nullptr, 0ull};

using PB16 = PBF16W;

}

#ifndef MLP_TU
#define MLP_TU 0
#endif
#if MLP_TU == 0 || MLP_TU == 1
int mlp_launch_proposal(const void* packed, int precision, const nerf_amd_samples& s, float* density, hipStream_t st) {
    if (precision == NERF_AMD_BF16)
        return launch<PB16, PropLayout, false, false, (MLP_RESIDENT_PROP ? PropResident::TOTAL : 0)>(proposal_kernel<PB16, false>, packed, s, density, st, NO_DUMP);
    return launch<PF32, PropLayout>(proposal_kernel<PF32, false>, packed, s, density, st, NO_DUMP);
}
#endif
#if MLP_TU == 0 || MLP_TU == 2
int mlp_launch_mip(const void* packed, int precision, const nerf_amd_samples& s, float* rgbo, hipStream_t st) {
    const FusedComposite off{nullptr, nullptr, nullptr, 0, 0.0f, 1.0f};
    if (s.ipe) {
        if (precision == NERF_AMD_BF16) return launch<PB16, MipLayout>(mip_kernel<PB16, false, true>, packed, s, rgbo, st, off, NO_DUMP);
        return launch<PF32, MipLayout>(mip_kernel<PF32, false, true>, packed, s, rgbo, st, off, NO_DUMP);
    }
    if (precision == NERF_AMD_BF16)
        return launch<PB16, MipLayout, false, false, (MLP_RESIDENT_MIP ? MipResident::TOTAL : 0)>(mip_kernel<PB16, false>, packed, s, rgbo, st, off, NO_DUMP);
    return launch<PF32, MipLayout>(mip_kernel<PF32, false>, packed, s, rgbo, st, off, NO_DUMP);
}
int mlp_launch_mip128(const void* packed, int precision, const nerf_amd_samples& s, float* rgbo, hipStream_t st) {
    if (precision == NERF_AMD_BF16) return launch<PB16, MipLayout128>(mip128_kernel<PB16>, packed, s, rgbo, st);
    return launch<PF32, MipLayout128>(mip128_kernel<PF32>, packed, s, rgbo, st);
}
int mlp_launch_mip_composite(const void* packed, int precision, const nerf_amd_samples& s, float* rgb, float* depth, float* weights,
                             int white_bkg, float near, float far, hipStream_t st) {
    const FusedComposite fc{rgb, depth, weights, white_bkg, near, far};
    if (precision == NERF_AMD_BF16) return launch<PB16, MipLayout>(mip_kernel<PB16, false, false, false, true>, packed, s, (float*)nullptr, st, fc, NO_DUMP);
    return launch<PF32, MipLayout>(mip_kernel<PF32, false, false, false, true>, packed, s, (float*)nullptr, st, fc, NO_DUMP);
}
#endif
#if MLP_TU == 0 || MLP_TU == 1
template <class P>
static int launch_proposal128(const void* packed, const nerf_amd_samples& s, float* density, hipStream_t st) {
    constexpr int TS = P::NW * P::NT * 32;
    const int64_t n_tiles = (s.M + TS - 1) / TS;
    if (n_tiles == 0) return 0;
    const size_t lds = lds_total_narrow();
    if (int e = allow_dynamic_lds(reinterpret_cast<const void*>(proposal128_kernel<P>), lds)) return e;
    hipLaunchKernelGGL(proposal128_kernel<P>, dim3(grid_for(n_tiles)), dim3(P::NW * 64), lds, st, packed, s, density);
    return (int)hipGetLastError();
}
int mlp_launch_proposal128(const void* packed, int precision, const nerf_amd_samples& s, float* density, hipStream_t st) {
    if (precision == NERF_AMD_BF16) return launch_proposal128<PBF16N>(packed, s, density, st);
    return launch_proposal128<PF32>(packed, s, density, st);
}
#endif
#if MLP_TU == 0 || MLP_TU == 1
size_t mlp_train_layer_stride(int precision, int64_t M) {
    const int64_t ts = (precision != NERF_AMD_F32) ? (int64_t)PB16::NW * PB16::NT * 32 : (int64_t)PF32::NW * PF32::NT * 32;
    const int64_t n_sub = ((M + ts - 1) / ts) * (ts / 32);
    return (size_t)n_sub * 16 * (precision != NERF_AMD_F32 ? 1024 : 2048);
}
size_t mlp_train_mask_stride(int precision, int64_t M) { return mlp_train_layer_stride(precision, M) / (16 * (precision != NERF_AMD_F32 ? 1024 : 2048)) * 1024; }
#else
size_t mlp_train_layer_stride(int precision, int64_t M);
size_t mlp_train_mask_stride(int precision, int64_t M);
#endif
static ActDump make_dump(void* dump, int precision, int64_t M, int slots) {
    const unsigned long long ls = mlp_train_layer_stride(precision, M);
    return ActDump{reinterpret_cast<char*>(dump), ls, reinterpret_cast<char*>(dump) + (size_t)slots * ls, (unsigned long long)mlp_train_mask_stride(precision, M)};
}
#if MLP_TU == 0 || MLP_TU == 1
int mlp_launch_proposal_train(const void* packed, int precision, const nerf_amd_samples& s, float* density, void* dump, hipStream_t st) {
    if (precision == NERF_AMD_BF16_F8) {
        const ActDump d8 = make_dump(dump, NERF_AMD_BF16, s.M, PROP_DUMP_SLOTS);
        return launch<PB16, PropLayout, true, true>(proposal_kernel<PB16, true, true>, packed, s, density, st, d8);
    }
    const ActDump d = make_dump(dump, precision, s.M, PROP_DUMP_SLOTS);
    if (precision == NERF_AMD_BF16) return launch<PBF16, PropLayout, true>(proposal_kernel<PBF16, true>, packed, s, density, st, d);
    return launch<PF32, PropLayout, true>(proposal_kernel<PF32, true>, packed, s, density, st, d);
}
#endif
#if MLP_TU == 0 || MLP_TU == 2
int mlp_launch_mip_train(const void* packed, int precision, const nerf_amd_samples& s, float* rgbo, void* dump, hipStream_t st) {
    const FusedComposite off{nullptr, nullptr, nullptr, 0, 0.0f, 1.0f};
    if (precision == NERF_AMD_BF16_F8) {
        const ActDump d8 = make_dump(dump, NERF_AMD_BF16, s.M, MIP_DUMP_SLOTS);
        if (s.ipe) return launch<PB16, MipLayout, true, true>(mip_kernel<PB16, true, true, true>, packed, s, rgbo, st, off, d8);
        return launch<PB16, MipLayout, true, true>(mip_kernel<PB16, true, false, true>, packed, s, rgbo, st, off, d8);
    }
    const ActDump d = make_dump(dump, precision, s.M, MIP_DUMP_SLOTS);
    if (s.ipe) {
        if (precision == NERF_AMD_BF16) return launch<PB16, MipLayout, true>(mip_kernel<PB16, true, true>, packed, s, rgbo, st, off, d);
        return launch<PF32, MipLayout, true>(mip_kernel<PF32, true, true>, packed, s, rgbo, st, off, d);
    }
    if (precision == NERF_AMD_BF16) return launch<PB16, MipLayout, true>(mip_kernel<PB16, true>, packed, s, rgbo, st, off, d);
    return launch<PF32, MipLayout, true>(mip_kernel<PF32, true>, packed, s, rgbo, st, off, d);
}

#endif
// ... 28 lines not shown
```

nerf_amd/csrc/pack_kernels.hip:

```cpp
#include "device_common.h"
#include "mlp_layout.h"

namespace {

enum { SEG_DMAP = 0, SEG_PE = 1, SEG_IDE = 2 };

struct PackLayer {
    const float* b;
    int rows;
    const float* w2; const float* b2; int rows2; int stride2;
    int nkg, nfb;
    int frag_start, bias_off;
    const float* seg_w[3];
    int seg_stride[3];
    int seg_kind[3], seg_nkg[3], seg_col[3], seg_L[3], seg_width[3];
    int trans;
    int seg_first[3];
};

constexpr int PACK_MAX_LAYERS = 24;
struct PackBatch { PackLayer L[PACK_MAX_LAYERS]; };

template <bool BF16>
__global__ void pack_layer_kernel(PackBatch B, char* __restrict__ stream, float* __restrict__ bias) {
    const PackLayer& L = B.L[blockIdx.y];
    const int n_elem = L.nfb * L.nkg * 512;
    for (int i = blockIdx.x * blockDim.x + threadIdx.x; i < n_elem; i += gridDim.x * blockDim.x) {
        const int e = i & 7, lane = (i >> 3) & 63, frag = i >> 9;
        const int grp = frag / (2 * L.nkg);
        int fb, kg;
        if (2 * grp + 1 < L.nfb) { const int r = frag - grp * 2 * L.nkg; kg = r >> 1; fb = 2 * grp + (r & 1); }
        else { fb = 2 * grp; kg = frag - 2 * grp * L.nkg; }
        const int row = 32 * fb + (lane & 31), h = lane >> 5;
        int seg = 0, lkg = kg;
        if (lkg >= L.seg_nkg[0]) { lkg -= L.seg_nkg[0]; seg = 1; if (lkg >= L.seg_nkg[1]) { lkg -= L.seg_nkg[1]; seg = 2; } }
        int col;
        if (L.seg_kind[seg] == SEG_PE) col = pe_slot_column(8 * lkg + e, h, L.seg_L[seg]);
        else if (L.seg_kind[seg] == SEG_IDE) col = ide_slot_column(8 * lkg + e, h);
        else col = dmap_feature(lkg, h, e);
        if (col >= L.seg_width[seg]) col = -1;
        float v = 0.0f;
        if (L.trans) {
            const int f = dmap_feature(lkg, h, e) - L.seg_first[seg];
            if (f >= 0 && f < L.seg_width[seg] && row < L.rows) v = L.seg_w[seg][(size_t)f * L.seg_stride[seg] + L.seg_col[seg] + row];
        } else if (col >= 0) {
            if (row < L.rows) v = L.seg_w[seg][(size_t)row * L.seg_stride[seg] + L.seg_col[seg] + col];
            else if (row < L.rows + L.rows2) v = L.w2[(size_t)(row - L.rows) * L.stride2 + L.seg_col[seg] + col];
        }
        const size_t f = (size_t)(L.frag_start + frag);
        if (BF16) reinterpret_cast<__bf16*>(stream + f * 1024)[lane * 8 + e] = (__bf16)v;
        else reinterpret_cast<float*>(stream + f * 2048)[(e >> 2) * 256 + lane * 4 + (e & 3)] = v;
    }
    const int n_b = (bias != nullptr) ? 32 * L.nfb : 0;
    for (int i = blockIdx.x * blockDim.x + threadIdx.x; i < n_b; i += gridDim.x * blockDim.x) {
        bias[L.bias_off + i] = (i < L.rows) ? L.b[i] : ((i < L.rows + L.rows2) ? L.b2[i - L.rows] : 0.0f);
    }
}

PackLayer make_layer(const float* w, const float* b, int rows, int in_f, int nkg, int nfb, int start, int bias_off) {
    PackLayer L{};
    L.b = b; L.rows = rows; L.nkg = nkg; L.nfb = nfb; L.frag_start = start; L.bias_off = bias_off;
    L.w2 = nullptr; L.b2 = nullptr; L.rows2 = 0; L.stride2 = 0;
    L.seg_w[2] = w; L.seg_stride[2] = in_f; L.seg_kind[2] = SEG_DMAP; L.seg_nkg[2] = 0; L.seg_col[2] = 0; L.seg_L[2] = 0; L.seg_width[2] = 0;
    L.seg_w[0] = w; L.seg_stride[0] = in_f; L.seg_kind[0] = SEG_DMAP; L.seg_nkg[0] = nkg; L.seg_col[0] = 0; L.seg_L[0] = 0;
    L.seg_width[0] = 16 * nkg;
    L.seg_w[1] = w; L.seg_stride[1] = in_f; L.seg_kind[1] = SEG_DMAP; L.seg_nkg[1] = 0; L.seg_col[1] = 0; L.seg_L[1] = 0;
    L.seg_width[1] = 0;
    return L;
}
void set_seg(PackLayer& L, int s, int kind, int nkg, int col, int pe_L, int width) {
    L.seg_kind[s] = kind; L.seg_nkg[s] = nkg; L.seg_col[s] = col; L.seg_L[s] = pe_L; L.seg_width[s] = width;
}

__global__ void fold_bottleneck_kernel(const float* __restrict__ w8, const float* __restrict__ b8, const float* __restrict__ wb,
                                       const float* __restrict__ bb, float* __restrict__ wf, float* __restrict__ bf) {
    const int i = blockIdx.x;
    const int j = threadIdx.x;
    float acc = 0.0f;
    for (int k = 0; k < 256; ++k) acc = __builtin_fmaf(w8[i * 283 + k], wb[k * 256 + j], acc);
    wf[i * 256 + j] = acc;
    if (j == 0) {
        float s = 0.0f;
        for (int k = 0; k < 256; ++k) s = __builtin_fmaf(w8[i * 283 + k], bb[k], s);
        bf[i] = s + b8[i];
    }
}

int launch_pack(const PackBatch& B, int n_layers, int precision, char* stream, float* bias, hipStream_t st) {
    int blocks = 1;
    for (int l = 0; l < n_layers; ++l) {
        const int n = B.L[l].nfb * B.L[l].nkg * 512;
        blocks = ((n + 255) / 256 > blocks) ? (n + 255) / 256 : blocks;
    }
    if (precision == NERF_AMD_BF16) hipLaunchKernelGGL(pack_layer_kernel<true>, dim3(blocks, n_layers), dim3(256), 0, st, B, stream, bias);
    else hipLaunchKernelGGL(pack_layer_kernel<false>, dim3(blocks, n_layers), dim3(256), 0, st, B, stream, bias);
    return (int)hipGetLastError();
}

}

int pack_proposal(int precision, const float* const* w, const float* const* b, void* packed, hipStream_t st) {
    using Lay = PropLayout;
    char* stream = reinterpret_cast<char*>(packed);
    float* bias = reinterpret_cast<float*>(stream + Lay::stream_bytes(precision));
    const int rows[5] = {256, 256, 256, 256, 1};
    const int inf[5] = {63, 256, 256, 256, 256};
    PackBatch B = {};
    for (int l = 0; l < 5; ++l) {
        PackLayer& L = B.L[l] = make_layer(w[l], b[l], rows[l], inf[l], Lay::NKG[l], Lay::NFB[l], Lay::START[l], Lay::BIAS_OFF[l]);
        if (l == 0) set_seg(L, 0, SEG_PE, 4, 0, 10, 63);
    }
    return launch_pack(B, 5, precision, stream, bias, st);
}

int pack_proposal128(int precision, const float* const* w, const float* const* b, void* packed, hipStream_t st) {
    using Lay = PropLayout128;
    char* stream = reinterpret_cast<char*>(packed);
    float* bias = reinterpret_cast<float*>(stream + Lay::stream_bytes(precision));
    const size_t frag = (precision == NERF_AMD_BF16) ? 1024 : 2048;
    if (int e = (int)hipMemsetAsync(stream + Lay::USED_FRAGS * frag, 0, (Lay::N_FRAGS - Lay::USED_FRAGS) * frag, st)) return e;
    const int rows[5] = {128, 128, 128, 128, 1};
    const int inf[5] = {63, 128, 128, 128, 128};
    PackBatch B = {};
    for (int l = 0; l < 5; ++l) {
        PackLayer& L = B.L[l] = make_layer(w[l], b[l], rows[l], inf[l], Lay::NKG[l], Lay::NFB[l], Lay::START[l], Lay::BIAS_OFF[l]);
        if (l == 0) set_seg(L, 0, SEG_PE, 4, 0, 10, 63);
    }
    return launch_pack(B, 5, precision, stream, bias, st);
}

int pack_mip(int precision, const float* const* w, const float* const* b, void* packed, hipStream_t st) {
    using Lay = MipLayout;
    char* stream = reinterpret_cast<char*>(packed);
    float* bias = reinterpret_cast<float*>(stream + Lay::stream_bytes(precision));
    float* wf = bias + Lay::N_BIAS;
    float* bf = wf + 128 * 256;
    hipLaunchKernelGGL(fold_bottleneck_kernel, dim3(128), dim3(256), 0, st, w[9], b[9], w[7], b[7], wf, bf);
    if (int e = (int)hipGetLastError()) return e;
    const float* lw[10] = {w[0], w[1], w[2], w[3], w[4], w[5], w[6], w[8], wf, w[10]};
    const float* lb[10] = {b[0], b[1], b[2], b[3], b[4], b[5], b[6], b[8], bf, b[10]};
    const int rows[10] = {256, 256, 256, 256, 256, 256, 256, 1, 128, 3};
    const int inf[10] = {63, 256, 256, 256, 319, 256, 256, 256, 256, 128};
    PackBatch B = {};
    for (int l = 0; l < 10; ++l) {
        PackLayer& L = B.L[l] = make_layer(lw[l], lb[l], rows[l], inf[l], Lay::NKG[l], Lay::NFB[l], Lay::START[l], Lay::BIAS_OFF[l]);
        if (l == 0) set_seg(L, 0, SEG_PE, 4, 0, 10, 63);
        if (l == 4) { set_seg(L, 0, SEG_PE, 4, 0, 10, 63); set_seg(L, 1, SEG_DMAP, 16, 63, 0, 256); }
        if (l == 8) {
            set_seg(L, 0, SEG_DMAP, 16, 0, 0, 256);
            set_seg(L, 1, SEG_PE, 2, 256, 4, 27);
            L.seg_w[1] = w[9]; L.seg_stride[1] = 283;
        }
    }
    return launch_pack(B, 10, precision, stream, bias, st);
}

int pack_mip128(int precision, const float* const* w, const float* const* b, void* packed, hipStream_t st) {
    using Lay = MipLayout128;
    char* stream = reinterpret_cast<char*>(packed);
    float* bias = reinterpret_cast<float*>(stream + Lay::stream_bytes(precision));
    float* wf = bias + Lay::N_BIAS;
    float* bf = wf + 128 * 256;
    hipLaunchKernelGGL(fold_bottleneck_kernel, dim3(128), dim3(256), 0, st, w[9], b[9], w[7], b[7], wf, bf);
    if (int e = (int)hipGetLastError()) return e;
    const float* lw[10] = {w[0], w[1], w[2], w[3], w[4], w[5], w[6], w[8], wf, w[10]};
    const float* lb[10] = {b[0], b[1], b[2], b[3], b[4], b[5], b[6], b[8], bf, b[10]};
    const int rows[10] = {128, 128, 128, 128, 128, 128, 256, 1, 128, 3};
    const int inf[10] = {63, 128, 128, 128, 191, 128, 128, 256, 256, 128};
    PackBatch B = {};
    for (int l = 0; l < 10; ++l) {
        PackLayer& L = B.L[l] = make_layer(lw[l], lb[l], rows[l], inf[l], Lay::NKG[l], Lay::NFB[l], Lay::START[l], Lay::BIAS_OFF[l]);
        if (l == 0) set_seg(L, 0, SEG_PE, 4, 0, 10, 63);
        if (l == 4) { set_seg(L, 0, SEG_PE, 4, 0, 10, 63); set_seg(L, 1, SEG_DMAP, 8, 63, 0, 128); }
        if (l == 8) {
            set_seg(L, 0, SEG_DMAP, 16, 0, 0, 256);
            set_seg(L, 1, SEG_PE, 2, 256, 4, 27);
            L.seg_w[1] = w[9]; L.seg_stride[1] = 283;
        }
    }
    return launch_pack(B, 10, precision, stream, bias, st);
}

int pack_ref(int precision, const float* const* w, const float* const* b, void* packed, hipStream_t st) {
    using Lay = RefLayout;
    char* stream = reinterpret_cast<char*>(packed);
    float* bias = reinterpret_cast<float*>(stream + Lay::stream_bytes(precision));
    const int tensor_of[18] = {0, 1, 2, 3, 4, 5, 6, 7, 8, 10, 11, 12, 13, 14, 15, 16, 17, 18};
    const int rows[18] = {256, 256, 256, 256, 256, 256, 256, 256, 128, 256, 256, 256, 256, 256, 256, 256, 256, 3};
    const int inf[18] = {63, 256, 256, 256, 319, 256, 256, 256, 256, 167, 256, 256, 256, 423, 256, 256, 256, 256};
    PackBatch B = {};
    for (int l = 0; l < 18; ++l) {
        const int t = tensor_of[l];
        PackLayer& L = B.L[l] = make_layer(w[t], b[t], rows[l], inf[l], Lay::NKG[l], Lay::NFB[l], Lay::START[l], Lay::BIAS_OFF[l]);
// ... 189 lines not shown
```

nerf_amd/ops.py:

```python
import ctypes as C
from typing import Optional, Sequence

import torch

from . import _lib
from ._lib import lib, check, Samples, F32, BF16, BF16_F8, NET_PROPOSAL, NET_MIP, NET_REF, NET_PROPOSAL_128, NET_MIP_128, PROP_W128, FINE_W128, ACT_RELU, ACT_IDENTITY, ACT_SOFTPLUS

_PRECISION_OVERRIDE = None


def set_precision(p: Optional[str]):
    global _PRECISION_OVERRIDE
    if p not in (None, "fp32", "bf16"):
        raise ValueError("precision must be None, 'fp32' or 'bf16'")
    _PRECISION_OVERRIDE = p


_TRAIN_DUMPS = __import__("os").environ.get("NERF_AMD_TRAIN_DUMPS", "bf16")


def set_train_dumps(fmt: str):
    global _TRAIN_DUMPS
    if fmt not in ("bf16", "fp8"):
        raise ValueError("train dumps: 'bf16' or 'fp8'")
    _TRAIN_DUMPS = fmt


def train_precision(precision: int) -> int:
    return BF16_F8 if (precision == BF16 and _TRAIN_DUMPS == "fp8") else precision


def current_precision() -> int:
    if _PRECISION_OVERRIDE is not None:
        return BF16 if _PRECISION_OVERRIDE == "bf16" else F32
    return BF16 if torch.is_autocast_enabled() else F32


_RAW_STREAM = getattr(torch._C, "_cuda_getCurrentRawStream", None)
_CUR_DEVICE = getattr(torch._C, "_cuda_getDevice", None)


def _stream() -> int:
    if _RAW_STREAM is not None and _CUR_DEVICE is not None:
        return _RAW_STREAM(_CUR_DEVICE())
    return torch.cuda.current_stream().cuda_stream


def _dev(t: torch.Tensor, name: str, dtype: torch.dtype = torch.float32) -> torch.Tensor:
    if not t.is_cuda:
        raise RuntimeError("nerf_amd: '%s' must live on the HIP device (got %s); there is no CPU path" % (name, t.device))
    if t.dtype != dtype:
        t = t.to(dtype)
    return t.contiguous()


def _ptr(t: Optional[torch.Tensor]):
    return None if t is None else C.c_void_p(t.data_ptr())


def _prop_prec(packed_prop: torch.Tensor, precision: int, packed_fine: Optional[torch.Tensor] = None) -> int:
    return int(precision) | int(getattr(packed_prop, "_nerf_amd_layout", 0)) | int(getattr(packed_fine, "_nerf_amd_layout", 0))


_PERSISTENT = __import__("os").environ.get("NERF_AMD_PERSISTENT_BUFFERS", "1") != "0"
_ARENA = {}
_ARENA_BUSY = {}
ARENA_STATS = {"persistent": 0, "fresh": 0, "grown": 0}


def set_persistent_buffers(on: bool) -> None:
    global _PERSISTENT
    _PERSISTENT = bool(on)
    if not on:
        release_buffers()


def release_buffers() -> None:
    _ARENA.clear()
    _ARENA_BUSY.clear()


def _arena_key(tag, device):
    return (device.index if device.index is not None else torch.cuda.current_device(), torch.cuda.current_stream(device).cuda_stream, tag)


def _arena_buffer(key, nbytes: int, device) -> torch.Tensor:
    buf = _ARENA.get(key)
    if buf is None or buf.numel() < nbytes:
        _ARENA.pop(key, None)
        buf = None
        buf = _ARENA[key] = torch.empty(nbytes, dtype=torch.uint8, device=device)
        ARENA_STATS["grown"] += 1
    return buf


def scratch(tag, nbytes: int, device) -> torch.Tensor:
    nbytes = int(nbytes)
    device = torch.device(device)
    if nbytes == 0 or not _PERSISTENT or torch.cuda.is_current_stream_capturing():
        ARENA_STATS["fresh"] += 1
        return torch.empty(nbytes, dtype=torch.uint8, device=device)
    ARENA_STATS["persistent"] += 1
    return _arena_buffer(_arena_key(tag, device), nbytes, device)[:nbytes]


class _Lease:
    __slots__ = ("key",)

    def __init__(self, key):
        self.key = key
        _ARENA_BUSY[key] = id(self)

    def __del__(self):
        try:
            if _ARENA_BUSY.get(self.key) == id(self):
                del _ARENA_BUSY[self.key]
        except Exception:
            pass


def leased(tag, nbytes: int, device) -> torch.Tensor:
    nbytes = int(nbytes)
    device = torch.device(device)
    if nbytes == 0 or not _PERSISTENT or torch.cuda.is_current_stream_capturing():
        ARENA_STATS["fresh"] += 1
        return torch.empty(nbytes, dtype=torch.uint8, device=device)
    key = _arena_key(tag, device)
    if key in _ARENA_BUSY:
        ARENA_STATS["fresh"] += 1
        return torch.empty(nbytes, dtype=torch.uint8, device=device)
    view = _arena_buffer(key, nbytes, device)[:nbytes]
    view._nerf_amd_lease = _Lease(key)
    ARENA_STATS["persistent"] += 1
    return view


def _raw(t: torch.Tensor, name: str) -> torch.Tensor:
    if t.is_cuda and t.dtype is torch.float32 and t.is_contiguous():
        return t
    return _dev(t.detach(), name)


def pack_weights(net: int, precision: int, weights: Sequence[torch.Tensor], biases: Sequence[torch.Tensor]) -> torch.Tensor:
    ws = [_raw(w, "weight") for w in weights]
    bs = [_raw(b, "bias") for b in biases]
    nbytes = lib.nerf_amd_packed_bytes(net, precision)
    packed = torch.empty(nbytes, dtype=torch.uint8, device=ws[0].device)
    n = len(ws)
    wp = (C.c_void_p * n)(*[w.data_ptr() for w in ws])
    bp = (C.c_void_p * n)(*[b.data_ptr() for b in bs])
    check(lib.nerf_amd_pack_weights(net, precision, wp, bp, n, _ptr(packed), _stream()), "nerf_amd_pack_weights")
    return packed


def _samples_pts(pts: torch.Tensor, stride: int, contract: bool = False) -> Samples:
    s = Samples()
    s.mode = 0
    s.M = pts.numel() // stride
    s.pts = pts.data_ptr()
    s.pts_stride = stride
    s.contract = int(bool(contract))
    return s


def samples_rays(rays: torch.Tensor, S: int, z: Optional[torch.Tensor] = None, z_base: Optional[torch.Tensor] = None,
                 u: Optional[torch.Tensor] = None, z_jitter: float = 0.0, contract: bool = False, ipe_radius: Optional[float] = None,
                 ipe_dir_norm: Optional[torch.Tensor] = None, seed: int = 0, rng_ray_offset: int = 0) -> Samples:
    s = Samples()
    s.contract = int(bool(contract))
    if ipe_radius is not None:
        if z is None or z.shape[-1] < S + 1 or ipe_dir_norm is None:
            raise ValueError("nerf_amd: integrated PE needs explicit z with S+1 depths per ray and ipe_dir_norm")
        s.ipe, s.ipe_radius, s.ipe_dir_norm = 1, float(ipe_radius), ipe_dir_norm.data_ptr()
    s.mode = 1
    s.S = S
    s.M = rays.shape[0] * S
    s.rays = rays.data_ptr()
    if z is not None:
        s.z = z.data_ptr()
        s.z_stride = z.shape[-1]
    else:
        s.z_base = z_base.data_ptr()
        if u is not None:
            s.u = u.data_ptr()
        else:
            s.rng_seed, s.rng_ray_offset = int(seed) & 0xFFFFFFFFFFFFFFFF, int(rng_ray_offset)
        s.z_jitter = z_jitter
        s.z_stride = S
    return s


def proposal_forward(packed: torch.Tensor, precision: int, pts: torch.Tensor, contract: bool = False) -> torch.Tensor:
    pts = _dev(pts, "pts")
    out = torch.empty(pts.shape[:-1], dtype=torch.float32, device=pts.device)
    if out.numel() == 0:
        return out
    s = _samples_pts(pts, 3, contract)
    check(lib.nerf_amd_proposal_forward(_ptr(packed), _prop_prec(packed, precision), C.byref(s), _ptr(out), _stream()), "nerf_amd_proposal_forward")
    return out


def proposal_forward_samples(packed, precision, s: Samples, shape, device) -> torch.Tensor:
    out = torch.empty(shape, dtype=torch.float32, device=device)
    check(lib.nerf_amd_proposal_forward(_ptr(packed), _prop_prec(packed, precision), C.byref(s), _ptr(out), _stream()), "nerf_amd_proposal_forward")
    return out


def mip_forward(packed: torch.Tensor, precision: int, pts: torch.Tensor, contract: bool = False) -> torch.Tensor:
    pts = _dev(pts, "pts")
    out = torch.empty(pts.shape[:-1] + (4,), dtype=torch.float32, device=pts.device)
    if out.numel() == 0:
        return out
    s = _samples_pts(pts, 6, contract)
    check(lib.nerf_amd_mip_forward(_ptr(packed), _prop_prec(None, precision, packed), C.byref(s), _ptr(out), _stream()), "nerf_amd_mip_forward")
    return out


def mip_forward_samples(packed, precision, s: Samples, shape, device) -> torch.Tensor:
    out = torch.empty(tuple(shape) + (4,), dtype=torch.float32, device=device)
    check(lib.nerf_amd_mip_forward(_ptr(packed), _prop_prec(None, precision, packed), C.byref(s), _ptr(out), _stream()), "nerf_amd_mip_forward")
    return out


def mip_forward_composite(packed, precision, rays: torch.Tensor, z: torch.Tensor, n_samples: int, white_bkg: bool, near: float,
                          far: float, want_depth: bool = True, want_weights: bool = False):
    N = rays.shape[0]
    dev = rays.device
    if int(getattr(packed, "_nerf_amd_layout", 0)) & FINE_W128:
        rgbo = mip_forward_samples(packed, precision, samples_rays(rays, n_samples, z=z), (N, n_samples), dev)
        rgb, w, depth, _ = composite(rgbo, z, rays, True, bool(white_bkg), ACT_RELU, (near, far), want_weights=want_weights)
        return rgb, (depth if want_depth else None), (w if want_weights else None)
    rgb = torch.empty((N, 3), dtype=torch.float32, device=dev)
    depth = torch.empty((N,), dtype=torch.float32, device=dev) if want_depth else None
    w = torch.empty((N, n_samples), dtype=torch.float32, device=dev) if want_weights else None
# ... 1041 lines not shown
```

Baseline: 9.584 million.

## Add three-tile proposal MLP kernel with AGPR parking and plain weight layout

Adds a BF16 inference variant of the proposal MLP that processes three 32-sample tiles per wave instead of two. It parks some hidden activations in accumulation registers (AGPRs) to stay within the register budget, and packs a second copy of the weights in a plain fragment order for a tile-major block schedule. The variant is on by default for the proposal network through a new render-tiles selector. The aim is more weight reuse per fragment load and fewer waves per sample, at the cost of register pressure, AGPR copy traffic and a packed blob twice the size.

Result: no change. 9.635 million, median of 6 (+0.5%).

```diff
diff --git a/include/nerf_amd.h b/include/nerf_amd.h
--- a/include/nerf_amd.h
+++ b/include/nerf_amd.h
@@ -24,6 +24,7 @@
 #define NERF_AMD_PROP_W128 0x100
 #define NERF_AMD_NET_MIP_128 4
 #define NERF_AMD_FINE_W128 0x200
+#define NERF_AMD_PROP_T3 0x400
 
 #define NERF_AMD_ACT_RELU     0
 #define NERF_AMD_ACT_IDENTITY 1
@@ -32,6 +33,8 @@
 const char* nerf_amd_last_error(void);
 int         nerf_amd_version(void);
 int         nerf_amd_device_info(int* n_cu, int* arch_is_gfx950);
+int         nerf_amd_set_render_tiles(int net, int tiles);
+int         nerf_amd_render_tiles(int net);
 
 typedef struct nerf_amd_samples {
     int32_t      mode;
diff --git a/nerf_amd/_lib.py b/nerf_amd/_lib.py
--- a/nerf_amd/_lib.py
+++ b/nerf_amd/_lib.py
@@ -12,6 +12,7 @@
 NET_PROPOSAL, NET_MIP, NET_REF, NET_PROPOSAL_128, NET_MIP_128 = 0, 1, 2, 3, 4
 FINE_W128 = 0x200
 PROP_W128 = 0x100
+PROP_T3 = 0x400
 ACT_RELU, ACT_IDENTITY, ACT_SOFTPLUS = 0, 1, 2
 SPACING_LINEAR, SPACING_DISPARITY = 0, 1
 SPACINGS = {"linear": SPACING_LINEAR, "disparity": SPACING_DISPARITY}
@@ -34,6 +35,8 @@
     "nerf_amd_version": (C.c_int, []),
     "nerf_amd_device_info": (C.c_int, [C.POINTER(C.c_int), C.POINTER(C.c_int)]),
     "nerf_amd_packed_bytes": (C.c_size_t, [C.c_int, C.c_int]),
+    "nerf_amd_set_render_tiles": (C.c_int, [C.c_int, C.c_int]),
+    "nerf_amd_render_tiles": (C.c_int, [C.c_int]),
     "nerf_amd_pack_weights": (C.c_int, [C.c_int, C.c_int, C.POINTER(c_void), C.POINTER(c_void), C.c_int, c_void, c_void]),
     "nerf_amd_proposal_forward": (C.c_int, [c_void, C.c_int, C.POINTER(Samples), c_void, c_void]),
     "nerf_amd_mip_forward": (C.c_int, [c_void, C.c_int, C.POINTER(Samples), c_void, c_void]),
diff --git a/nerf_amd/_packed.py b/nerf_amd/_packed.py
--- a/nerf_amd/_packed.py
+++ b/nerf_amd/_packed.py
@@ -92,9 +92,15 @@
     def _narrow_layout(self) -> bool:
         return False
 
-    def _pack_now(self, precision: int, narrow: bool = False) -> torch.Tensor:
+    def _render_layout(self, precision: int, narrow: bool, wide: bool) -> int:
+        if (self._net_id == ops.NET_PROPOSAL and not narrow and not wide and not self.training and int(precision) == ops.BF16
+                and ops.render_tiles(ops.NET_PROPOSAL) == 3):
+            return ops.PROP_T3
+        return 0
+
+    def _pack_now(self, precision: int, narrow: bool = False, layout: int = 0) -> torch.Tensor:
         ws, bs = self.kernel_params()
-        return ops.pack_weights(self._net_id, precision, ws, bs)
+        return ops.pack_weights(self._net_id, precision, ws, bs, layout=layout)
 
     def packed_backward(self, precision: int) -> torch.Tensor:
         return ops.pack_weights_backward(self._net_id, precision, self.kernel_params()[0])
@@ -117,10 +123,11 @@
             cache.clear()
             return self._pack_now(precision, narrow)
         key = self._packed_key()
-        hit = cache.get((precision, narrow))
+        layout = self._render_layout(precision, narrow, wide)
+        hit = cache.get((precision, narrow, layout))
         if hit is None or hit[0] != key:
-            blob = self._pack_now(precision, narrow)
-            cache[(precision, narrow)] = (key, blob)
+            blob = self._pack_now(precision, narrow, layout) if layout else self._pack_now(precision, narrow)
+            cache[(precision, narrow, layout)] = (key, blob)
             return blob
         return hit[1]
 
diff --git a/nerf_amd/addtional.py b/nerf_amd/addtional.py
--- a/nerf_amd/addtional.py
+++ b/nerf_amd/addtional.py
@@ -122,9 +122,9 @@
     def _narrow_layout(self) -> bool:
         return self.hidden_unit <= 128
 
-    def _pack_now(self, precision: int, narrow: bool = False) -> torch.Tensor:
+    def _pack_now(self, precision: int, narrow: bool = False, layout: int = 0) -> torch.Tensor:
         if not narrow:
-            return super()._pack_now(precision)
+            return super()._pack_now(precision, layout=layout)
         ws, bs = self.kernel_params(self._NARROW_SHAPES)
         blob = ops.pack_weights(ops.NET_PROPOSAL_128, precision, ws, bs)
         blob._nerf_amd_layout = ops.PROP_W128
diff --git a/nerf_amd/csrc/capi.hip b/nerf_amd/csrc/capi.hip
--- a/nerf_amd/csrc/capi.hip
+++ b/nerf_amd/csrc/capi.hip
@@ -6,6 +6,7 @@
 #include "mlp_layout.h"
 
 int mlp_launch_proposal(const void*, int, const nerf_amd_samples&, float*, hipStream_t);
+int mlp_launch_proposal_t3(const void*, const nerf_amd_samples&, float*, hipStream_t);
 int mlp_launch_proposal128(const void*, int, const nerf_amd_samples&, float*, hipStream_t);
 int mlp_launch_mip(const void*, int, const nerf_amd_samples&, float*, hipStream_t);
 int mlp_launch_mip128(const void*, int, const nerf_amd_samples&, float*, hipStream_t);
@@ -47,7 +48,7 @@
                          hipStream_t);
 int bwd_launch_adam(float* const*, const float* const*, float* const*, float* const*, const long long*, int, float*, double, const double*, double,
                     double, double, float, hipStream_t);
-int pack_proposal(int, const float* const*, const float* const*, void*, hipStream_t);
+int pack_proposal(int, const float* const*, const float* const*, void*, hipStream_t, int plain);
 int pack_proposal128(int, const float* const*, const float* const*, void*, hipStream_t);
 int pack_mip128(int, const float* const*, const float* const*, void*, hipStream_t);
 int pack_mip(int, const float* const*, const float* const*, void*, hipStream_t);
@@ -173,8 +174,21 @@
     return NERF_AMD_OK;
 }
 
+static int g_render_tiles[2] = {3, 2};
+int nerf_amd_set_render_tiles(int net, int tiles) {
+    if (net != NERF_AMD_NET_PROPOSAL && net != NERF_AMD_NET_MIP) return fail(NERF_AMD_EINVAL, "no render-tile selector for this network");
+    if (tiles != 2 && !(tiles == 3 && net == NERF_AMD_NET_PROPOSAL))
+        return fail(NERF_AMD_EUNSUPPORTED, "render tiles: 2 or 3 for the proposal kernel, 2 for the fine kernel (its three-tile form does not fit the register file)");
+    g_render_tiles[net == NERF_AMD_NET_MIP] = tiles;
+    return NERF_AMD_OK;
+}
+int nerf_amd_render_tiles(int net) { return (net == NERF_AMD_NET_PROPOSAL || net == NERF_AMD_NET_MIP) ? g_render_tiles[net == NERF_AMD_NET_MIP] : 0; }
+
 size_t nerf_amd_packed_bytes(int net, int precision) {
-    if (bad_prec(precision)) return 0;
+    const int lflags = precision & ~0xff;
+    precision &= 0xff;
+    if (bad_prec(precision) || (lflags & ~NERF_AMD_PROP_T3)) return 0;
+    if (lflags & NERF_AMD_PROP_T3) return (net == NERF_AMD_NET_PROPOSAL && precision == NERF_AMD_BF16) ? 2 * PropLayout::packed_bytes(precision) : 0;
     if (net == NERF_AMD_NET_PROPOSAL) return PropLayout::packed_bytes(precision);
     if (net == NERF_AMD_NET_MIP) return MipLayout::packed_bytes(precision);
     if (net == NERF_AMD_NET_REF) return RefLayout::packed_bytes(precision);
@@ -186,12 +200,18 @@
     return (flags & NERF_AMD_FINE_W128) ? mlp_launch_mip128(packed, precision, s, rgbo, st) : mlp_launch_mip(packed, precision, s, rgbo, st);
 }
 static int launch_proposal_any(int flags, const void* packed, int precision, const nerf_amd_samples& s, float* density, hipStream_t st) {
+    if ((flags & NERF_AMD_PROP_T3) && !(flags & NERF_AMD_PROP_W128) && precision == NERF_AMD_BF16 && g_render_tiles[0] == 3)
+        return mlp_launch_proposal_t3(reinterpret_cast<const char*>(packed) + PropLayout::packed_bytes(precision), s, density, st);
     return (flags & NERF_AMD_PROP_W128) ? mlp_launch_proposal128(packed, precision, s, density, st) : mlp_launch_proposal(packed, precision, s, density, st);
 }
 
 int nerf_amd_pack_weights(int net, int precision, const float* const* weights, const float* const* biases, int n_tensors,
                           void* packed, void* stream) {
-    if (bad_prec(precision)) return fail(NERF_AMD_EINVAL, "unknown precision");
+    const int lflags = precision & ~0xff;
+    precision &= 0xff;
+    if (bad_prec(precision) || (lflags & ~NERF_AMD_PROP_T3)) return fail(NERF_AMD_EINVAL, "unknown precision");
+    if ((lflags & NERF_AMD_PROP_T3) && (net != NERF_AMD_NET_PROPOSAL || precision != NERF_AMD_BF16))
+        return fail(NERF_AMD_EINVAL, "NERF_AMD_PROP_T3: the bf16 blob of NERF_AMD_NET_PROPOSAL only");
     if (!weights || !biases || !packed) return fail(NERF_AMD_EINVAL, "NULL argument");
     const int want = (net == NERF_AMD_NET_PROPOSAL || net == NERF_AMD_NET_PROPOSAL_128) ? 5
                      : ((net == NERF_AMD_NET_MIP || net == NERF_AMD_NET_MIP_128) ? 11 : (net == NERF_AMD_NET_REF ? 20 : -1));
@@ -199,7 +219,10 @@
     if (n_tensors != want) return fail(NERF_AMD_EINVAL, "wrong number of weight tensors for this network");
     for (int i = 0; i < want; ++i)
         if (!weights[i] || !biases[i]) return fail(NERF_AMD_EINVAL, "NULL weight or bias tensor");
-    const int e = net == NERF_AMD_NET_PROPOSAL ? pack_proposal(precision, weights, biases, packed, S(stream))
+    if (lflags & NERF_AMD_PROP_T3)
+        if (int e2 = pack_proposal(precision, weights, biases, reinterpret_cast<char*>(packed) + PropLayout::packed_bytes(precision), S(stream), 1))
+            return hip_status(e2, "nerf_amd_pack_weights");
+    const int e = net == NERF_AMD_NET_PROPOSAL ? pack_proposal(precision, weights, biases, packed, S(stream), 0)
                   : net == NERF_AMD_NET_PROPOSAL_128 ? pack_proposal128(precision, weights, biases, packed, S(stream))
                   : net == NERF_AMD_NET_MIP_128 ? pack_mip128(precision, weights, biases, packed, S(stream))
                   : (net == NERF_AMD_NET_MIP ? pack_mip(precision, weights, biases, packed, S(stream))
@@ -210,7 +233,7 @@
 int nerf_amd_proposal_forward(const void* packed, int precision, const nerf_amd_samples* src, float* density, void* stream) {
     const int lflags = precision & ~0xff;
     precision &= 0xff;
-    if (bad_prec(precision) || (lflags & ~NERF_AMD_PROP_W128)) return fail(NERF_AMD_EINVAL, "unknown precision");
+    if (bad_prec(precision) || (lflags & ~(NERF_AMD_PROP_W128 | NERF_AMD_PROP_T3))) return fail(NERF_AMD_EINVAL, "unknown precision");
     if (int c = check_samples(src, false)) return c;
     if (src->M == 0) return NERF_AMD_OK;
     if (!packed || !density) return fail(NERF_AMD_EINVAL, "NULL argument");
@@ -718,7 +741,7 @@
                          float* depth, float* weights, void* workspace, void* stream) {
     const int lflags = precision & ~0xff;
     precision &= 0xff;
-    if (bad_prec(precision) || (lflags & ~(NERF_AMD_PROP_W128 | NERF_AMD_FINE_W128))) return fail(NERF_AMD_EINVAL, "unknown precision");
+    if (bad_prec(precision) || (lflags & ~(NERF_AMD_PROP_W128 | NERF_AMD_FINE_W128 | NERF_AMD_PROP_T3))) return fail(NERF_AMD_EINVAL, "unknown precision");
     if ((lflags & NERF_AMD_FINE_W128) && camera && camera->ipe) return fail(NERF_AMD_EINVAL, "the 128-wide fine layout has no integrated-PE kernel: pack the network 256-wide");
     if (N < 0 || n_fine < 1 || n_fine > 1023) return fail(NERF_AMD_EINVAL, "bad N or n_fine");
     if (N == 0) return NERF_AMD_OK;
@@ -821,7 +844,7 @@
     precision &= 0xff;
     float gn, gf;
     if (int e = check_spacing(spacing, near, far, &gn, &gf)) return e;
-    if (bad_prec(precision) || (lflags & ~(NERF_AMD_PROP_W128 | NERF_AMD_FINE_W128))) return fail(NERF_AMD_EINVAL, "unknown precision");
+    if (bad_prec(precision) || (lflags & ~(NERF_AMD_PROP_W128 | NERF_AMD_FINE_W128 | NERF_AMD_PROP_T3))) return fail(NERF_AMD_EINVAL, "unknown precision");
     if ((lflags & NERF_AMD_FINE_W128) && camera && camera->ipe) return fail(NERF_AMD_EINVAL, "the 128-wide fine layout has no integrated-PE kernel: pack the network 256-wide");
     if (N < 0 || n_fine < 1 || n_fine > 1023) return fail(NERF_AMD_EINVAL, "bad N or n_fine");
     constexpr int C = 64;
@@ -894,7 +917,7 @@
                              float* rgb, float* depth, float* normal_img, void* workspace, void* stream) {
     const int lflags = precision & ~0xff;
     precision &= 0xff;
-    if (bad_prec(precision) || (lflags & ~NERF_AMD_PROP_W128) || bad_ref_flags(ref_flags)) return fail(NERF_AMD_EINVAL, "unknown precision or ref_flags");
+    if (bad_prec(precision) || (lflags & ~(NERF_AMD_PROP_W128 | NERF_AMD_PROP_T3)) || bad_ref_flags(ref_flags)) return fail(NERF_AMD_EINVAL, "unknown precision or ref_flags");
     if (N < 0 || n_fine < 1 || n_fine > 1023) return fail(NERF_AMD_EINVAL, "bad N or n_fine");
     if (N == 0) return NERF_AMD_OK;
     if (!packed_prop || !packed_ref || !z_base || !rgb || !workspace) return fail(NERF_AMD_EINVAL, "NULL argument");
diff --git a/nerf_amd/csrc/mlp_core.h b/nerf_amd/csrc/mlp_core.h
--- a/nerf_amd/csrc/mlp_core.h
+++ b/nerf_amd/csrc/mlp_core.h
@@ -13,6 +13,7 @@
     static constexpr int PREC = NERF_AMD_BF16;
     static constexpr int NW = MLP_NW_BF16;
     static constexpr int NT = 1;
+    static constexpr bool ONE_BLOCK = false;
     static constexpr int FRAG_BYTES = 1024;
     static constexpr int FPC = MLP_CHUNK_BYTES / FRAG_BYTES;
     using AReg = bf16x8;
@@ -46,6 +47,7 @@
         return r;
     }
     static constexpr bool FAST_PE = true;
+    static DEVINL BReg park(const BReg& r, bool, int) { return r; }
     static constexpr int BREG_LDS = 1024;
     static DEVINL void stash(uint32_t addr, const BReg& r) { *reinterpret_cast<bf16x8*>(smem + addr) = r; }
     static DEVINL BReg unstash(uint32_t addr) { return *reinterpret_cast<const bf16x8*>(smem + addr); }
@@ -65,11 +67,28 @@
     static constexpr int NT = 3;
 };
 
+struct PBF16W3 : PBF16 {
+    static constexpr int NW = 4;
+    static constexpr int NT = 3;
+    static constexpr bool ONE_BLOCK = true;
+    static constexpr int DEPTH = 2;
+    static DEVINL BReg to_agpr(const BReg& r) {
+        typedef __attribute__((ext_vector_type(4))) uint32_t u32x4_;
+        const u32x4_ d = __builtin_bit_cast(u32x4_, r);
+        u32x4_ o;
+#pragma unroll
+        for (int i = 0; i < 4; ++i) { uint32_t x; asm("v_accvgpr_write_b32 %0, %1" : "=a"(x) : "v"((uint32_t)d[i])); o[i] = x; }
+        return __builtin_bit_cast(BReg, o);
+    }
+    static DEVINL BReg park(const BReg& r, bool is_b, int t) { return (!is_b || t >= 2) ? to_agpr(r) : r; }
+};
+
 struct PF32 {
     using BReg = f32x8;
     static constexpr int PREC = NERF_AMD_F32;
     static constexpr int NW = MLP_NW_F32;
     static constexpr int NT = 1;
+    static constexpr bool ONE_BLOCK = false;
     static constexpr int FRAG_BYTES = 2048;
     static constexpr int FPC = MLP_CHUNK_BYTES / FRAG_BYTES;
     struct AReg { f32x4 lo, hi; };
@@ -98,6 +117,7 @@
         return r;
     }
     static constexpr bool FAST_PE = false;
+    static DEVINL BReg park(const BReg& r, bool, int) { return r; }
     static constexpr int BREG_LDS = 2048;
     static DEVINL void stash(uint32_t addr, const BReg& r) {
         f32x4 lo = {r[0], r[1], r[2], r[3]}, hi = {r[4], r[5], r[6], r[7]};
@@ -445,16 +465,82 @@
         return d;
     }
 }
+template <class P, int NKG, int FRAG0, int KG, bool MORE, int FB, class WS, class InF, class OutF, class Prev>
+DEVINL void block_k(WS& ws, f32x16 (&acc)[P::NT], f32x16& nb, uint32_t next_bias, InF& in, OutF& out, const Prev& prev) {
+    if constexpr (MORE && KG == NKG - 2) {
+        static_assert(P::NT == 3 && NKG >= 4, "tile-major block tail");
+        const typename P::AReg a0 = ws.template next<FRAG0 + KG>();
+        const typename P::AReg a1 = ws.template next<FRAG0 + KG + 1>();
+        acc[0] = P::template mma_pos<1>(a0, in(KG, 0), acc[0]);
+        acc[0] = P::template mma_pos<2>(a1, in(KG + 1, 0), acc[0]);
+        acc[1] = P::template mma_pos<1>(a0, in(KG, 1), acc[1]);
+        acc[1] = P::template mma_pos<2>(a1, in(KG + 1, 1), acc[1]);
+        out(FB, 0, acc[0], 0);
+        acc[2] = P::template mma_pos<1>(a0, in(KG, 2), acc[2]);
+        out(FB, 0, acc[0], 1);
+        acc[2] = P::template mma_pos<2>(a1, in(KG + 1, 2), acc[2]);
+    } else if constexpr (KG < NKG) {
+        typename P::BReg b[P::NT];
+#pragma unroll
+        for (int t = 0; t < P::NT; ++t) b[t] = in(KG, t);
+        const typename P::AReg a = ws.template next<FRAG0 + KG>();
+        constexpr int POS = (KG == 0) ? 0 : ((KG == NKG - 1) ? 2 : 1);
+#pragma unroll
+        for (int t = 0; t < P::NT; ++t) acc[t] = P::template mma_pos<POS>(a, b[t], acc[t]);
+        emit_step<NKG, KG>(prev);
+        if constexpr (MORE && KG == (NKG > 3 ? NKG - 3 : 0)) nb = load_bias(next_bias);
+        block_k<P, NKG, FRAG0, KG + 1, MORE, FB>(ws, acc, nb, next_bias, in, out, prev);
+    }
+}
+template <int NT, int TLO, int THI, class Prev, int S = 0>
+DEVINL void flush_tiles(const Prev& prev) {
+    if constexpr (S < Prev::NSL) {
+        if constexpr (S % NT >= TLO && S % NT < THI) prev.template emit<S>();
+        flush_tiles<NT, TLO, THI, Prev, S + 1>(prev);
+    }
+}
+template <class Prev, int NT, int T0>
+struct TileTail {
+    static constexpr int NSL = (NT - T0) * 2;
+    const Prev& p;
+    template <int S> DEVINL void emit() const { p.template emit<(S / (NT - T0)) * NT + T0 + S % (NT - T0)>(); }
+};
+template <class P, int NKG, int NFB, int START, int FB, class WS, class InF, class OutF, class Prev>
+DEVINL auto dense1_block(WS& ws, uint32_t bias_lane, const f32x16& cb, InF& in, OutF& out, const Prev& prev) {
+    constexpr int FRAG0 = START + FB * NKG;
+    constexpr bool MORE = FB + 1 < NFB;
+    Deferred<P, FB, 1> d;
+#pragma unroll
+    for (int t = 0; t < P::NT; ++t) d.acc[0][t] = cb;
+    f32x16 nb;
+    if constexpr (FB > 0) {
+        static_assert(Prev::NSL == 2 * P::NT, "prev = the block before this one");
+        flush_tiles<P::NT, 1, P::NT - 1>(prev);
+        block_k<P, NKG, FRAG0, 0, MORE, FB>(ws, d.acc[0], nb, bias_lane + 128 * (FB + 1), in, out, TileTail<Prev, P::NT, P::NT - 1>{prev});
+    } else {
+        block_k<P, NKG, FRAG0, 0, MORE, FB>(ws, d.acc[0], nb, bias_lane + 128 * (FB + 1), in, out, prev);
+    }
+    if constexpr (MORE) return dense1_block<P, NKG, NFB, START, FB + 1>(ws, bias_lane, nb, in, out, prev_of(d, out));
+    else return d;
+}
+template <class P, int NFB, bool ONE = (P::ONE_BLOCK && NFB > 1)> struct LastGroup { using type = Deferred<P, 2 * ((NFB - 1) / 2), 2 - NFB % 2>; };
+template <class P, int NFB> struct LastGroup<P, NFB, true> { using type = Deferred<P, NFB - 1, 1>; };
+
 template <class P, int NKG, int NFB, int START, bool ZB = false, class WS, class InF, class OutF, class Prev>
 DEVINL auto dense(WS& ws, uint32_t bias_lds, InF&& in, OutF&& out, const Prev& prev) {
     static_assert(START % P::DEPTH == 0 && (NKG * NFB) % P::DEPTH == 0, "layers must start on a prefetch-queue boundary");
     const uint32_t bias_lane = bias_lds + 16 * (lane_id() >> 5);
+    if constexpr (P::ONE_BLOCK && NFB > 1) {
+        static_assert(!ZB && !has_group_hook<OutF>::value, "one-block chains: the inference layers");
+        return dense1_block<P, NKG, NFB, START, 0>(ws, bias_lane, load_bias(bias_lane), in, out, prev);
+    } else {
     f32x16 cb[2];
     if constexpr (!ZB) {
         cb[0] = load_bias(bias_lane);
         if constexpr (NFB > 1) cb[1] = load_bias(bias_lane + 128);
     }
     return dense_group<P, NKG, NFB, START, 0, ZB>(ws, bias_lane, cb, in, out, prev);
-}
-
-}
+    }
+}
+
+}
diff --git a/nerf_amd/csrc/mlp_kernels.hip b/nerf_amd/csrc/mlp_kernels.hip
--- a/nerf_amd/csrc/mlp_kernels.hip
+++ b/nerf_amd/csrc/mlp_kernels.hip
@@ -329,7 +329,9 @@
     using L = PropLayout;
     using BReg = typename P::BReg;
     constexpr int FPC = P::FPC;
-    constexpr bool RES = MLP_RESIDENT_PROP && same_type<P, PBF16W>::value && !TRAIN;
+    constexpr bool T3 = same_type<P, PBF16W3>::value;
+    static_assert(!T3 || !TRAIN, "PBF16W3 is an inference policy");
+    constexpr bool RES = ((MLP_RESIDENT_PROP && same_type<P, PBF16W>::value) || T3) && !TRAIN;
     using R = typename conditional_type<RES, PropResident::R, NoResident>::type;
     using WS = typename conditional_type<RES, WeightStream<P, PropResident::NSLOT, R, PropResident::RES>, WeightStream<P, MLP_NSLOT>>::type;
     constexpr uint32_t bias0 = RES ? PropResident::BIAS : MLP_RING_BYTES;
@@ -348,13 +350,18 @@
     for (int64_t tile = blockIdx.x; tile < n_tiles; tile += gridDim.x) {
         int64_t m[NT];
         BReg enc[NT][4];
-        if constexpr (NT == 2 && P::FAST_PE) {
+        if constexpr (NT >= 2 && P::FAST_PE) {
             m[0] = tile * TS + (wave * NT) * 32 + j;
             m[1] = m[0] + 32;
             const int64_t mo = h ? m[1] : m[0];
             const Sample sm = fetch_sample(s, mo < s.M ? mo : s.M - 1, false);
             encode_pair<P, 10, 4>(sm.x, sm.y, sm.z, enc[0], enc[1]);
             half_swap_groups<4>(enc[0], enc[1]);
+            if constexpr (NT > 2) {
+                m[2] = m[0] + 64;
+                const Sample s2 = fetch_sample(s, m[2] < s.M ? m[2] : s.M - 1, false);
+                encode<P, 10, 4>(s2.x, s2.y, s2.z, h, enc[NT - 1]);
+            }
             if constexpr (TRAIN) {
 #pragma unroll
                 for (int t = 0; t < NT; ++t)
@@ -377,7 +384,7 @@
         int lay = 0, lay_pend = 0;
         const int64_t sub0 = tile * (TS / 32) + wave * NT;
         auto put = [&](BReg (&buf)[NT][16], int layer, int fb, int t, const f32x16& acc, int half) {
-            buf[t][2 * fb + half] = to_breg_half<P, true>(acc, half);
+            buf[t][2 * fb + half] = P::park(to_breg_half<P, true>(acc, half), &buf == &b, t);
             if constexpr (TRAIN) {
                 dump_hidden<P, F8>(dump, sacc, layer, sub0 + t, t, 2 * fb + half, lane, buf[t][2 * fb + half]);
                 mask_or<P>(macc, layer, t, 2 * fb + half, lane, buf[t][2 * fb + half]);
@@ -388,7 +395,7 @@
         auto OA_pend = [&](int fb, int t, const f32x16& acc, int half) { put(a, lay_pend, fb, t, acc, half); };
         auto OB_pend = [&](int fb, int t, const f32x16& acc, int half) { put(b, lay_pend, fb, t, acc, half); };
         auto IN_A = [&](int kg, int t) -> BReg { return a[t][kg]; };
-        Deferred<P, 6, 2> d = dense<P, 4, 8, L::START[0]>(ws, bias0 + L::BIAS_OFF[0] * 4,
+        typename LastGroup<P, 8>::type d = dense<P, 4, 8, L::START[0]>(ws, bias0 + L::BIAS_OFF[0] * 4,
             [&](int kg, int t) -> BReg { return enc[t][kg]; }, OA, NoPrev{});
         static_assert(same_stream_shape<R, FPC>(L::START[1], L::START[3], 128 + P::DEPTH), "chunk parity (in stream space) of the shared a -> b instance");
         auto IN_B = [&](int kg, int t) -> BReg { return b[t][kg]; };
@@ -397,6 +404,7 @@
             lay_pend = lay; lay = 1 + 2 * r;
             d = dense<P, 16, 8, L::START[1]>(ws, bias0 + (L::BIAS_OFF[1] + r * 512) * 4, IN_A, OB, prev_of(d, OA_pend));
             if constexpr (TRAIN) mask_flush<P, F8>(dump, macc, lay_pend, sub0, lane, sacc);
+            if constexpr (T3) { if (r == 1) break; }
             if (r == 0) {
                 lay_pend = lay; lay = 2;
                 d = dense<P, 16, 8, L::START[2]>(ws, bias0 + L::BIAS_OFF[2] * 4, IN_B, OA, prev_of(d, OB_pend));
@@ -409,8 +417,10 @@
         dense<P, 16, 1, L::START[4]>(ws, bias0 + L::BIAS_OFF[4] * 4, IN_B, OH, prev_of(d, OB_pend)).flush(OH);
         if constexpr (TRAIN) mask_flush<P, F8>(dump, macc, lay_pend, sub0, lane, sacc);
 #pragma unroll
-        for (int t = 0; t < NT; ++t)
-            if (h == 0 && m[t] < s.M) density[m[t]] = dens[t];
+        for (int t = 0; t < NT; ++t) {
+            const int64_t mt = T3 ? tile * TS + (wave * NT + t) * 32 + j : m[t];
+            if (h == 0 && mt < s.M) density[mt] = dens[t];
+        }
     }
     ws.drain();
 }
@@ -1148,6 +1158,9 @@
         return launch<PB16, PropLayout, false, false, (MLP_RESIDENT_PROP ? PropResident::TOTAL : 0)>(proposal_kernel<PB16, false>, packed, s, density, st, NO_DUMP);
     return launch<PF32, PropLayout>(proposal_kernel<PF32, false>, packed, s, density, st, NO_DUMP);
 }
+int mlp_launch_proposal_t3(const void* packed, const nerf_amd_samples& s, float* density, hipStream_t st) {
+    return launch<PBF16W3, PropLayout, false, false, PropResident::TOTAL>(proposal_kernel<PBF16W3, false>, packed, s, density, st, NO_DUMP);
+}
 #endif
 #if MLP_TU == 0 || MLP_TU == 2
 int mlp_launch_mip(const void* packed, int precision, const nerf_amd_samples& s, float* rgbo, hipStream_t st) {
diff --git a/nerf_amd/csrc/pack_kernels.hip b/nerf_amd/csrc/pack_kernels.hip
--- a/nerf_amd/csrc/pack_kernels.hip
+++ b/nerf_amd/csrc/pack_kernels.hip
@@ -16,6 +16,7 @@
     int seg_kind[3], seg_nkg[3], seg_col[3], seg_L[3], seg_width[3];
     int trans;
     int seg_first[3];
+    int plain;
 };
 
 constexpr int PACK_MAX_LAYERS = 24;
@@ -29,7 +30,8 @@
         const int e = i & 7, lane = (i >> 3) & 63, frag = i >> 9;
         const int grp = frag / (2 * L.nkg);
         int fb, kg;
-        if (2 * grp + 1 < L.nfb) { const int r = frag - grp * 2 * L.nkg; kg = r >> 1; fb = 2 * grp + (r & 1); }
+        if (L.plain) { fb = frag / L.nkg; kg = frag - fb * L.nkg; }
+        else if (2 * grp + 1 < L.nfb) { const int r = frag - grp * 2 * L.nkg; kg = r >> 1; fb = 2 * grp + (r & 1); }
         else { fb = 2 * grp; kg = frag - 2 * grp * L.nkg; }
         const int row = 32 * fb + (lane & 31), h = lane >> 5;
         int seg = 0, lkg = kg;
@@ -99,7 +101,7 @@
 
 }
 
-int pack_proposal(int precision, const float* const* w, const float* const* b, void* packed, hipStream_t st) {
+int pack_proposal(int precision, const float* const* w, const float* const* b, void* packed, hipStream_t st, int plain) {
     using Lay = PropLayout;
     char* stream = reinterpret_cast<char*>(packed);
     float* bias = reinterpret_cast<float*>(stream + Lay::stream_bytes(precision));
@@ -109,6 +111,7 @@
     for (int l = 0; l < 5; ++l) {
         PackLayer& L = B.L[l] = make_layer(w[l], b[l], rows[l], inf[l], Lay::NKG[l], Lay::NFB[l], Lay::START[l], Lay::BIAS_OFF[l]);
         if (l == 0) set_seg(L, 0, SEG_PE, 4, 0, 10, 63);
+        L.plain = plain;
     }
     return launch_pack(B, 5, precision, stream, bias, st);
 }
diff --git a/nerf_amd/ops.py b/nerf_amd/ops.py
--- a/nerf_amd/ops.py
+++ b/nerf_amd/ops.py
@@ -4,7 +4,7 @@
 import torch
 
 from . import _lib
-from ._lib import lib, check, Samples, F32, BF16, BF16_F8, NET_PROPOSAL, NET_MIP, NET_REF, NET_PROPOSAL_128, NET_MIP_128, PROP_W128, FINE_W128, ACT_RELU, ACT_IDENTITY, ACT_SOFTPLUS
+from ._lib import lib, check, Samples, F32, BF16, BF16_F8, NET_PROPOSAL, NET_MIP, NET_REF, NET_PROPOSAL_128, NET_MIP_128, PROP_W128, FINE_W128, PROP_T3, ACT_RELU, ACT_IDENTITY, ACT_SOFTPLUS
 
 _PRECISION_OVERRIDE = None
 
@@ -141,15 +141,31 @@
     return _dev(t.detach(), name)
 
 
-def pack_weights(net: int, precision: int, weights: Sequence[torch.Tensor], biases: Sequence[torch.Tensor]) -> torch.Tensor:
+def set_render_tiles(prop: Optional[int] = None, fine: Optional[int] = None) -> None:
+    if prop is not None:
+        check(lib.nerf_amd_set_render_tiles(NET_PROPOSAL, int(prop)), "nerf_amd_set_render_tiles")
+    if fine is not None:
+        check(lib.nerf_amd_set_render_tiles(NET_MIP, int(fine)), "nerf_amd_set_render_tiles")
+
+
+def render_tiles(net: int) -> int:
+    return int(lib.nerf_amd_render_tiles(net))
+
+
+def pack_weights(net: int, precision: int, weights: Sequence[torch.Tensor], biases: Sequence[torch.Tensor], layout: int = 0) -> torch.Tensor:
     ws = [_raw(w, "weight") for w in weights]
     bs = [_raw(b, "bias") for b in biases]
+    precision = int(precision) | int(layout)
     nbytes = lib.nerf_amd_packed_bytes(net, precision)
+    if nbytes == 0:
+        raise ValueError("nerf_amd: no packed layout for network %d with precision / layout flags 0x%x" % (net, precision))
     packed = torch.empty(nbytes, dtype=torch.uint8, device=ws[0].device)
     n = len(ws)
     wp = (C.c_void_p * n)(*[w.data_ptr() for w in ws])
     bp = (C.c_void_p * n)(*[b.data_ptr() for b in bs])
     check(lib.nerf_amd_pack_weights(net, precision, wp, bp, n, _ptr(packed), _stream()), "nerf_amd_pack_weights")
+    if layout:
+        packed._nerf_amd_layout = int(layout)
     return packed
 
 
```
